# tingliu/glia

Hardware: AMD Instinct MI355X
Metric: region_merges_per_sec (higher is better)
Workload: dtype u32 labels / f32 image / f64 statistics and features

## Files before the change

glia_amd/csrc/api.cpp:

```cpp
#include <algorithm>
#include <atomic>
#include <chrono>
#include <cmath>
#include <cstdio>
#include <cstdlib>
#include <cstring>
#include <limits>
#include <mutex>
#include <unordered_map>

#include "bc_features.hpp"
#include "forest.hpp"
#include "rmap_order.hpp"
#include "hmt_internal.hpp"

namespace glia {

static thread_local std::string g_err;
void set_error(const std::string& msg) { g_err = msg; }

static const char* const kOptionKeys[] = {"GLIA_HMT_PB_WINDOW", "GLIA_HMT_PB_BATCH", "GLIA_HMT_WINCAP", "GLIA_HMT_REBASE", "GLIA_HMT_HORIZON",
                                          "GLIA_HMT_FORCE_TREE", "GLIA_HMT_HELPERS", "GLIA_HMT_TRACE", "GLIA_HMT_LIBM", "GLIA_HMT_BC_NOCOMMON",
                                          "GLIA_HMT_BC_GENERIC", "GLIA_HMT_DEBUG", "GLIA_HMT_MAXITERS", "GLIA_HMT_MINCAP"};
static std::mutex g_opt_mu;
static std::unordered_map<std::string, std::string> g_opt;
static bool g_opt_init = false;
static void opt_init_locked() {
  if (g_opt_init) return;
  for (const char* k : kOptionKeys) if (const char* e = getenv(k)) g_opt[k] = e;
  g_opt_init = true;
}
static bool opt_known(const char* key) { for (const char* k : kOptionKeys) if (!strcmp(k, key)) return true; return false; }
bool option(const char* key, std::string* value) {
  std::lock_guard<std::mutex> lock(g_opt_mu);
  opt_init_locked();
  auto it = g_opt.find(key);
  if (it == g_opt.end()) return false;
  if (value) *value = it->second;
  return true;
}
int set_option(const char* key, const char* value) {
  if (!key || !opt_known(key)) { set_error(std::string("set_option: unknown option ") + (key ? key : "(null)")); return GLIA_HMT_ERR_ARG; }
  std::lock_guard<std::mutex> lock(g_opt_mu);
  opt_init_locked();
  if (value) g_opt[key] = value; else g_opt.erase(key);
  return GLIA_HMT_OK;
}

static float ceil_f32(double d) {
  if (std::isinf(d) || std::isnan(d)) return (float)d;
  float f = (float)d;
  if ((double)f < d) f = std::nextafterf(f, std::numeric_limits<float>::infinity());
  return f;
}
static float floor_f32(double d) {
  if (std::isinf(d) || std::isnan(d)) return (float)d;
  float f = (float)d;
  if ((double)f > d) f = std::nextafterf(f, -std::numeric_limits<float>::infinity());
  return f;
}
static uint32_t next_pow2(uint64_t v) {
  uint64_t p = 1;
  while (p < v) p <<= 1;
  return (uint32_t)std::min<uint64_t>(p, 1ull << 31);
}

HistSpec make_hist_spec(int bins, double lo, double hi) {
  HistSpec h;
  h.bins = bins;
  double interval = (hi - lo) / bins;
  double b = 0.0;
  for (int i = 0; i < GLIA_HMT_MAX_BINS; ++i) {
    if (i < bins) { b = (i == 0) ? interval : b + interval; h.fb[i] = ceil_f32(b); }
    else h.fb[i] = std::numeric_limits<float>::infinity();
  }
  h.lo_f = floor_f32(lo);
  h.hi_f = ceil_f32(hi);
  return h;
}


static LibmSel probe_host_libm() {
  std::vector<double> xs;
  uint64_t s = 0x9E3779B97F4A7C15ull;
  auto next = [&]() { s ^= s << 13; s ^= s >> 7; s ^= s << 17; return s; };
  for (int i = 0; i < 6000; ++i) { const uint64_t n = 1 + next() % 100000, c = 1 + next() % n; xs.push_back((double)c / (double)n); }
  for (int i = 0; i < 3000; ++i) xs.push_back(1.0 + ((double)(int64_t)(next() % 2000001) - 1000000.0) * 1e-7);
  for (int i = 0; i < 3000; ++i) xs.push_back(std::ldexp(1.0 + (double)(next() >> 12) * 0x1p-52, (int)(next() % 120) - 60));
  for (int e = -1074; e < 1024; e += 37) xs.push_back(std::ldexp(1.0, e));
  LibmSel sel = {kLibmDevice, kLibmDevice, kLibmDevice};
  bool l2 = true, ls = true, lf = true, ps = true, pf = true;
  for (double x : xs) {
    volatile double vx = x;
    const double h2 = std::log2(vx), h1 = std::log(vx);
    l2 = l2 && glibc::as_u64(h2) == glibc::as_u64(glibc::log2_sse2(x));
    ls = ls && glibc::as_u64(h1) == glibc::as_u64(glibc::log_sse2(x));
    lf = lf && glibc::as_u64(h1) == glibc::as_u64(glibc::log_fma(x));
  }
  for (int i = 0; i < 12000; ++i) {
    const double x = i < 4000 ? (double)(i + 1) : (double)(1 + next() % (i < 8000 ? (1ull << 24) : (1ull << 40)));
    volatile double vx = x, vy = 1.5;
    const uint64_t h = glibc::as_u64(std::pow(vx, vy));
    ps = ps && h == glibc::as_u64(glibc::pow_sse2(x, 1.5));
    pf = pf && h == glibc::as_u64(glibc::pow_fma(x, 1.5));
  }
  if (l2) sel.log2_variant = kLibmSse2;
  if (lf) sel.log_variant = kLibmFma; else if (ls) sel.log_variant = kLibmSse2;
  if (pf) sel.pow_variant = kLibmFma; else if (ps) sel.pow_variant = kLibmSse2;
  std::string ov;
  if (option("GLIA_HMT_LIBM", &ov)) {
    const char* e = ov.c_str();
    const int v = !strcmp(e, "sse2") ? kLibmSse2 : !strcmp(e, "fma") ? kLibmFma : kLibmDevice;
    sel.log_variant = v; sel.log2_variant = v == kLibmFma ? kLibmSse2 : v; sel.pow_variant = v;
  }
  return sel;
}

}

namespace glia {
GLIA_DECLARE_GREEDY_BC(greedy_bc) {
  auto* fn = &greedy_bc_generic;
  const bool common = cfg.K == 1 && cfg.n_region == 1 && cfg.n_rlabel == 0 && cfg.n_boundary == 1 && !cfg.use_hist && !cfg.use_log &&
                      !cfg.use_simple && !option("GLIA_HMT_BC_NOCOMMON");
  if (cfg.libm_log2 == kLibmSse2 && cfg.libm_log == kLibmFma && cfg.libm_pow == kLibmFma) fn = common ? &greedy_bc_fma_common : &greedy_bc_fma;
  else if (cfg.libm_log2 == kLibmSse2 && cfg.libm_log == kLibmSse2 && cfg.libm_pow == kLibmSse2) fn = common ? &greedy_bc_sse2_common : &greedy_bc_sse2;
  if (option("GLIA_HMT_BC_GENERIC")) fn = &greedy_bc_generic;
  const int rc = fn(rag, cfg, clf, stream, req, out);
  return req.init_only ? rc : finish_merge_order(rc, out->order.data(), out->n, (uint32_t)rag.R, stream);
}
}

using namespace glia;

#include "api_types.hpp"

static std::atomic<int> g_live_contexts{0};

static int free_tables(glia_hmt_ctx* c) {
  if (c->rkeys) GLIA_HIP_TRY(hipFree(c->rkeys));
  if (c->rrec) GLIA_HIP_TRY(hipFree(c->rrec));
  if (c->pkeys) GLIA_HIP_TRY(hipFree(c->pkeys));
  if (c->prec) GLIA_HIP_TRY(hipFree(c->prec));
  c->rkeys = nullptr; c->rrec = nullptr; c->pkeys = nullptr; c->prec = nullptr;
  c->rcap = c->pcap = 0;
  return GLIA_HMT_OK;
}

static int ensure_tables(glia_hmt_ctx* c, uint32_t rcap, uint32_t pcap) {
  if (rcap <= c->rcap && pcap <= c->pcap) return GLIA_HMT_OK;
  rcap = std::max(rcap, c->rcap);
  pcap = std::max(pcap, c->pcap);
  int rc = free_tables(c);
  if (rc) return rc;
  GLIA_HIP_TRY(hipMalloc(&c->rkeys, sizeof(uint32_t) * (size_t)rcap));
  GLIA_HIP_TRY(hipMalloc(&c->rrec, sizeof(uint32_t) * kRegionWords * (size_t)rcap));
  GLIA_HIP_TRY(hipMalloc(&c->pkeys, sizeof(unsigned long long) * (size_t)pcap));
  GLIA_HIP_TRY(hipMalloc(&c->prec, sizeof(uint32_t) * kPairWords * (size_t)pcap));
  GLIA_HIP_TRY(hipMemsetAsync(c->rkeys, 0, sizeof(uint32_t) * (size_t)rcap, c->stream));
  GLIA_HIP_TRY(hipMemsetAsync(c->rrec, 0, sizeof(uint32_t) * kRegionWords * (size_t)rcap, c->stream));
  GLIA_HIP_TRY(hipMemsetAsync(c->pkeys, 0, sizeof(unsigned long long) * (size_t)pcap, c->stream));
  GLIA_HIP_TRY(hipMemsetAsync(c->prec, 0, sizeof(uint32_t) * kPairWords * (size_t)pcap, c->stream));
  c->rcap = rcap;
  c->pcap = pcap;
  return GLIA_HMT_OK;
}

static int clear_tables(glia_hmt_ctx* c) {
  GLIA_HIP_TRY(hipMemsetAsync(c->rkeys, 0, sizeof(uint32_t) * (size_t)c->rcap, c->stream));
  GLIA_HIP_TRY(hipMemsetAsync(c->rrec, 0, sizeof(uint32_t) * kRegionWords * (size_t)c->rcap, c->stream));
  GLIA_HIP_TRY(hipMemsetAsync(c->pkeys, 0, sizeof(unsigned long long) * (size_t)c->pcap, c->stream));
  GLIA_HIP_TRY(hipMemsetAsync(c->prec, 0, sizeof(uint32_t) * kPairWords * (size_t)c->pcap, c->stream));
  return GLIA_HMT_OK;
}

extern "C" {
// ... 427 lines not shown
int glia_hmt_rag_from_arrays(glia_hmt_ctx* c, const glia_hmt_rag* like, int64_t n_regions, const uint32_t* d_region_label,
                             const uint32_t* d_region_rec, int64_t n_pairs, const uint32_t* d_pair_a, const uint32_t* d_pair_b,
                             const uint32_t* d_pair_rec, glia_hmt_rag** out) {
  if (!c || !like || !out || n_regions < 0 || n_pairs < 0) { set_error("rag_from_arrays: invalid argument"); return GLIA_HMT_ERR_ARG; }
  GLIA_HIP_TRY(hipSetDevice(c->device));
  glia_hmt_rag* rag = new glia_hmt_rag(*like);
  rag->ctx = c;
  rag->d_folded = nullptr; rag->vol = VolumeRef();
  rag->arr = RagArrays();
  rag->arr.R = n_regions; rag->arr.P = n_pairs;
  auto dup = [&](uint32_t** dst, const uint32_t* src, size_t n) -> int {
    GLIA_HIP_TRY(hipMalloc(dst, sizeof(uint32_t) * (n ? n : 1)));
    if (n) GLIA_HIP_TRY(hipMemcpyAsync(*dst, src, sizeof(uint32_t) * n, hipMemcpyDeviceToDevice, c->stream));
    return GLIA_HMT_OK;
  };
  int rc;
  if ((rc = dup(&rag->arr.d_rlabel, d_region_label, (size_t)n_regions)) || (rc = dup(&rag->arr.d_rrec, d_region_rec, (size_t)n_regions * kRegionWords)) ||
      (rc = dup(&rag->arr.d_pa, d_pair_a, (size_t)n_pairs)) || (rc = dup(&rag->arr.d_pb, d_pair_b, (size_t)n_pairs)) ||
      (rc = dup(&rag->arr.d_prec, d_pair_rec, (size_t)n_pairs * kPairWords))) { glia_hmt_rag_free(rag); return rc; }
  rag->arr.K = 1; rag->arr.c_rrec[0] = rag->arr.d_rrec; rag->arr.c_prec[0] = rag->arr.d_prec;
  for (int k = 0; k < kMaxChannels; ++k) rag->arr.c_bins[k] = like->arr.c_bins[k];
  rag->arr.c_bins[0] = rag->bins;
  GLIA_HIP_TRY(hipStreamSynchronize(c->stream));
  *out = rag;
  return GLIA_HMT_OK;
}

void glia_hmt_rag_free(glia_hmt_rag* r) {
  if (!r) return;
  (void)hipSetDevice(r->ctx->device);
  (void)hipFree(r->arr.d_rlabel); (void)hipFree(r->arr.d_rrec);
  (void)hipFree(r->arr.d_pa); (void)hipFree(r->arr.d_pb); (void)hipFree(r->arr.d_prec);
  for (int k = 1; k < r->arr.K; ++k) { (void)hipFree(r->arr.c_rrec[k]); (void)hipFree(r->arr.c_prec[k]); }
  if (r->arr.d_pv_off) (void)hipFree(r->arr.d_pv_off);
  if (r->arr.d_pv) (void)hipFree(r->arr.d_pv);
  if (r->d_folded) (void)hipFree(r->d_folded);
  delete r;
}

int64_t glia_hmt_rag_num_regions(const glia_hmt_rag* r) { return r ? r->arr.R : -1; }
int64_t glia_hmt_rag_num_pairs(const glia_hmt_rag* r) { return r ? r->arr.P : -1; }

int glia_hmt_rag_last_pass(const glia_hmt_rag* r, double* ms, double* bytes) {
  if (!r) return GLIA_HMT_ERR_ARG;
  if (ms) *ms = r->pass_ms;
  if (bytes) *bytes = r->alg_bytes;
  return GLIA_HMT_OK;
}

static double dword(const uint32_t* w) { double d; std::memcpy(&d, w, 8); return d; }

int glia_hmt_rag_export_regions(const glia_hmt_rag* r, uint32_t* h_label, int64_t* h_count, int64_t* h_border,
                                int64_t* h_lo, int64_t* h_hi, double* h_sum, double* h_sumsq, double* h_min,
                                double* h_max, int64_t* h_hist, int64_t* h_first) {
  if (!r) return GLIA_HMT_ERR_ARG;
  GLIA_HIP_TRY(hipSetDevice(r->ctx->device));
  const int64_t R = r->arr.R;
  std::vector<uint32_t> lab(R), rec((size_t)R * kRegionWords);
  if (R) {
    GLIA_HIP_TRY(hipMemcpy(lab.data(), r->arr.d_rlabel, sizeof(uint32_t) * R, hipMemcpyDeviceToHost));
    GLIA_HIP_TRY(hipMemcpy(rec.data(), r->arr.d_rrec, sizeof(uint32_t) * kRegionWords * R, hipMemcpyDeviceToHost));
  }
  for (int64_t i = 0; i < R; ++i) {
    const uint32_t* w = &rec[(size_t)i * kRegionWords];
    if (h_label) h_label[i] = lab[i];
    if (h_count) h_count[i] = w[R_CNT];
    if (h_border) h_border[i] = w[R_BORDER];
    for (int d = 0; d < 3; ++d) {
      if (h_lo) h_lo[3 * i + d] = (int64_t)(0x7fffffffu - w[R_LO + d]);
      if (h_hi) h_hi[3 * i + d] = (int64_t)w[R_HI + d] - 1;
    }
    if (h_sum) h_sum[i] = dword(&w[R_SUM]);
    if (h_sumsq) h_sumsq[i] = dword(&w[R_SQ]);
    if (h_min) h_min[i] = (double)ord_float(~w[R_MIN]);
    if (h_max) h_max[i] = (double)ord_float(w[R_MAX]);
    if (h_hist) for (int b = 0; b < r->bins; ++b) h_hist[i * r->bins + b] = w[R_HIST + b];
    if (h_first) { unsigned long long f; std::memcpy(&f, &w[R_FIRST], 8); h_first[i] = (int64_t)~f; }
  }
  return GLIA_HMT_OK;
}

int glia_hmt_rag_export_pairs(const glia_hmt_rag* r, uint32_t* h_a, uint32_t* h_b, int64_t* h_count, double* h_sum,
                              double* h_sumsq, double* h_min, double* h_max, int64_t* h_hist, int64_t* h_thr) {
  if (!r) return GLIA_HMT_ERR_ARG;
  GLIA_HIP_TRY(hipSetDevice(r->ctx->device));
  const int64_t P = r->arr.P;
  std::vector<uint32_t> a(P), b(P), rec((size_t)P * kPairWords);
  if (P) {
    GLIA_HIP_TRY(hipMemcpy(a.data(), r->arr.d_pa, sizeof(uint32_t) * P, hipMemcpyDeviceToHost));
    GLIA_HIP_TRY(hipMemcpy(b.data(), r->arr.d_pb, sizeof(uint32_t) * P, hipMemcpyDeviceToHost));
    GLIA_HIP_TRY(hipMemcpy(rec.data(), r->arr.d_prec, sizeof(uint32_t) * kPairWords * P, hipMemcpyDeviceToHost));
  }
  for (int64_t i = 0; i < P; ++i) {
    const uint32_t* w = &rec[(size_t)i * kPairWords];
    if (h_a) h_a[i] = a[i];
    if (h_b) h_b[i] = b[i];
    if (h_count) h_count[i] = w[P_CNT];
    if (h_sum) h_sum[i] = dword(&w[P_SUM]);
    if (h_sumsq) h_sumsq[i] = dword(&w[P_SQ]);
    if (h_min) h_min[i] = (double)ord_float(~w[P_MIN]);
    if (h_max) h_max[i] = (double)ord_float(w[P_MAX]);
    if (h_hist) for (int k = 0; k < r->bins; ++k) h_hist[i * r->bins + k] = w[P_HIST + k];
    if (h_thr) for (int k = 0; k < r->nthr; ++k) h_thr[i * r->nthr + k] = w[P_THR + k];
  }
  return GLIA_HMT_OK;
}

static int order_to_keys(const glia_hmt_rag* rag, const MergeResult& res, const char* who, bool contour_keys, int64_t capacity,
                         uint32_t* h_order, double* h_sal, int64_t* n_merges) {
  const int64_t R = rag->arr.R, n = res.n;
  if (n > capacity) { set_error(std::string(who) + ": output capacity too small"); return GLIA_HMT_ERR_CAPACITY; }
  std::vector<uint32_t> lab((size_t)R);
  GLIA_HIP_TRY(hipMemcpy(lab.data(), rag->arr.d_rlabel, sizeof(uint32_t) * R, hipMemcpyDeviceToHost));
  uint32_t maxKey = lab[R - 1];
  if (contour_keys) GLIA_HIP_TRY(hipMemcpy(&maxKey, rag->arr.d_pa + (rag->arr.P - 1), sizeof(uint32_t), hipMemcpyDeviceToHost));
  for (int64_t i = 0; i < 3 * n; ++i) {
    const uint32_t id = res.order[i];
    h_order[i] = id < (uint32_t)R ? lab[id] : maxKey + 1u + (id - (uint32_t)R);
  }
  std::copy(res.sal.begin(), res.sal.begin() + n, h_sal);
  *n_merges = n;
  return GLIA_HMT_OK;
}

int glia_hmt_merge_order_pb(glia_hmt_ctx* c, glia_hmt_rag* rag, int type, uint32_t* h_order, double* h_sal,
                            int64_t capacity, int64_t* n_merges) {
  if (!c || !rag || !h_order || !h_sal || !n_merges || rag->ctx != c) {
    set_error("merge_order_pb: invalid argument");
    return GLIA_HMT_ERR_ARG;
  }
  if (type == 3 && rag->only_contour) {
    set_error("merge_order_pb: the median x min-size linkage needs region sizes (only_contour = 0)");
    return GLIA_HMT_ERR_ARG;
  }
  if ((type == 1 || type == 3) && !rag->vol.lab && !rag->arr.d_pv_off) {
    set_error("merge_order_pb: median linkage needs the volumes the RAG was built from (whole-volume build) or a map that carries its "
              "boundary values (glia_hmt_rag_build_distributed with with_values)");
    return GLIA_HMT_ERR_UNSUPPORTED;
  }
  if (type != 1 && type != 2 && type != 3) {
    set_error("Error: unsupported boundary stats type...");
    return GLIA_HMT_ERR_ARG;
  }
  GLIA_HIP_TRY(hipSetDevice(c->device));
  *n_merges = 0;
  if (rag->arr.R == 0 || rag->arr.P == 0) return GLIA_HMT_OK;
  PbRequest req;
  if (type == 1 || type == 3) req.median_of = &rag->vol;
  req.size_weight = type == 3;
  MergeResult res;
  const int rc = greedy_mean(rag->arr, c->stream, req, &res);
  if (rc) return rc;
  rag->ms_table = res.ms_table; rag->ms_loop = res.ms_loop; rag->n_scored = res.n_scored;
  return order_to_keys(rag, res, "merge_order_pb", rag->only_contour, capacity, h_order, h_sal, n_merges);
}

static int upload_forest(const HostForest& hf, glia_hmt_forest* f, int slot, hipStream_t stream) {
  std::vector<PackedNode> nodes;
  std::vector<int> roots;
  int rc = pack_forest(hf, &nodes, &roots);
  if (rc) return rc;
  PackedNode* d_nodes = nullptr;
  int* d_roots = nullptr;
  GLIA_HIP_TRY(hipMalloc(&d_nodes, sizeof(PackedNode) * nodes.size()));
  f->allocs.push_back(d_nodes);
  GLIA_HIP_TRY(hipMalloc(&d_roots, sizeof(int) * roots.size()));
  f->allocs.push_back(d_roots);
  GLIA_HIP_TRY(hipMemcpyAsync(d_nodes, nodes.data(), sizeof(PackedNode) * nodes.size(), hipMemcpyHostToDevice, stream));
  GLIA_HIP_TRY(hipMemcpyAsync(d_roots, roots.data(), sizeof(int) * roots.size(), hipMemcpyHostToDevice, stream));
  std::vector<PackedTriple> lines;
  std::vector<int> proots;
  rc = pack_forest_triples(hf, &lines, &proots);
  if (rc) return rc;
  PackedTriple* d_lines = nullptr;
  int* d_proots = nullptr;
  GLIA_HIP_TRY(hipMalloc(&d_lines, sizeof(PackedTriple) * lines.size()));
  f->allocs.push_back(d_lines);
  GLIA_HIP_TRY(hipMalloc(&d_proots, sizeof(int) * proots.size()));
  f->allocs.push_back(d_proots);
  GLIA_HIP_TRY(hipMemcpyAsync(d_lines, lines.data(), sizeof(PackedTriple) * lines.size(), hipMemcpyHostToDevice, stream));
  GLIA_HIP_TRY(hipMemcpyAsync(d_proots, proots.data(), sizeof(int) * proots.size(), hipMemcpyHostToDevice, stream));
  GLIA_HIP_TRY(hipStreamSynchronize(stream));
  f->dc.f[slot].ntree = hf.ntree; f->dc.f[slot].nrnodes = hf.nrnodes; f->dc.f[slot].nnodes = (int)nodes.size();
  f->dc.f[slot].nodes = d_nodes; f->dc.f[slot].root = d_roots;
  f->dc.f[slot].triples = d_lines; f->dc.f[slot].troot = d_proots;
  if (hf.max_var > f->max_var) f->max_var = hf.max_var;
  return GLIA_HMT_OK;
}

int glia_hmt_forest_load(glia_hmt_ctx* c, int n_models, const char* const* paths, int predict_label,
                         const double* dist, glia_hmt_forest** out) {
  if (!c || !paths || !out || (n_models != 1 && n_models != 3)) {
    set_error("forest_load: one model, or three models with distributor arguments, expected");
    return GLIA_HMT_ERR_ARG;
  }
  if (n_models == 3 && !dist) { set_error("Error: model distributor needs 3 arguments..."); return GLIA_HMT_ERR_ARG; }
  GLIA_HIP_TRY(hipSetDevice(c->device));
  glia_hmt_forest* f = new glia_hmt_forest;
  f->device = c->device;
  memset(&f->dc, 0, sizeof(f->dc));
  f->dc.kind = 0; f->dc.n_models = n_models;
  if (dist) {
    f->dc.dim0 = (int)dist[0]; f->dc.dim1 = (int)dist[1]; f->dc.threshold = dist[2];
    if (f->dc.dim0 < 0 || f->dc.dim1 < 0) { delete f; set_error("forest_load: negative distributor dimension"); return GLIA_HMT_ERR_ARG; }
    f->max_var = std::max(f->dc.dim0, f->dc.dim1);
  }
  for (int i = 0; i < n_models; ++i) {
    HostForest hf;
    int rc = load_forest_file(paths[i], predict_label, &hf);
    if (rc == GLIA_HMT_OK) rc = upload_forest(hf, f, i, c->stream);
    if (rc) { glia_hmt_forest_free(f); return rc; }
  }
  *out = f;
  return GLIA_HMT_OK;
}

int glia_hmt_forest_file_parse(const char* path, int predict_label, int* ntree, int* nrnodes, int* nclass,
                               double* h_split, int* h_meta, int64_t capacity_nodes) {
  if (!path || !ntree || !nrnodes || !nclass) { set_error("forest_file_parse: invalid argument"); return GLIA_HMT_ERR_ARG; }
  HostForest hf;
  int rc = load_forest_file(path, predict_label, &hf);
  if (rc) return rc;
  *ntree = hf.ntree; *nrnodes = hf.nrnodes; *nclass = hf.nclass;
  const int64_t nodes = (int64_t)hf.ntree * hf.nrnodes;
  if (h_split || h_meta) {
    if (nodes > capacity_nodes) { set_error("forest_file_parse: capacity too small"); return GLIA_HMT_ERR_CAPACITY; }
    if (h_split) memcpy(h_split, hf.split.data(), sizeof(double) * nodes);
    if (h_meta) memcpy(h_meta, hf.meta.data(), sizeof(int) * 4 * nodes);
  }
  return GLIA_HMT_OK;
}

int glia_hmt_forest_stub(glia_hmt_ctx* c, int feature_index, glia_hmt_forest** out) {
  if (!c || !out || feature_index < 0) { set_error("forest_stub: invalid argument"); return GLIA_HMT_ERR_ARG; }
  glia_hmt_forest* f = new glia_hmt_forest;
  f->device = c->device;
  memset(&f->dc, 0, sizeof(f->dc));
  f->dc.kind = 1; f->dc.n_models = 1; f->dc.stub_index = feature_index; f->max_var = feature_index;
  *out = f;
  return GLIA_HMT_OK;
}

void glia_hmt_forest_free(glia_hmt_forest* f) {
  if (!f) return;
  (void)hipSetDevice(f->device);
  for (void* p : f->allocs) (void)hipFree(p);
  delete f;
}

static inline double sdivide_host(double l, double r) { return std::fabs(r) >= 2.22e-16 ? l / r : 0.0; }

static bool make_bc_cfg(const glia_hmt_rag* rag, BcCfg* c) {
  if (!rag->has_cfg) return false;
  const glia_hmt_feat_config& g = rag->cfg;
  memset(c, 0, sizeof(*c));
  c->D = rag->dim; c->T = g.n_thresholds; c->bins = rag->bins;
  c->K = rag->arr.K;
  for (int k = 0; k < kMaxChannels; ++k) c->cbins[k] = k < rag->arr.K ? rag->arr.c_bins[k] : 0;
  c->n_region = g.n_region; c->n_rlabel = g.n_rlabel; c->n_boundary = g.n_boundary;
  for (int i = 0; i < kMaxListed; ++i) { c->rc[i] = rag->map_region[i]; c->lc[i] = rag->map_rlabel[i]; c->bc[i] = rag->map_boundary[i]; }
  c->use_log = g.use_log_shape; c->use_simple = g.use_simple_features; c->use_hist = g.use_histogram_features;
  c->norm_area = g.normalizing_area; c->norm_len = g.normalizing_length;
  c->rfdim = bc_rf_dim(*c); c->bfdim = bc_bf_dim(*c); c->fdim = bc_feat_dim(*c);
  c->libm_log2 = rag->ctx->libm.log2_variant; c->libm_log = rag->ctx->libm.log_variant; c->libm_pow = rag->ctx->libm.pow_variant;
  return true;
}

static int median_extra_cols(const glia_hmt_rag* rag, const BcCfg& c) {
  if (!rag->cfg.use_median_features) return 0;
  return c.use_simple ? c.n_boundary : 4 * c.n_region + 4 * c.n_boundary;
}
static int refuse_median_in_loop(const glia_hmt_rag* rag, const char* who) {
  if (!rag->has_cfg || !rag->cfg.use_median_features) return GLIA_HMT_OK;
  set_error(std::string(who) + ": the GLIA_USE_MEDIAN_AS_FEATS layout (type/feat.hxx:677-722) is implemented for a given merge order only (glia_hmt_bc_feat): "
            "inside the greedy loop every contraction changes the value multisets of its regions and boundary sets");
  return GLIA_HMT_ERR_UNSUPPORTED;
}

int glia_hmt_feat_dim(const glia_hmt_rag* rag) {
  BcCfg c;
  if (!rag || !make_bc_cfg(rag, &c)) return -1;
  return c.fdim + median_extra_cols(rag, c);
}

static int bc_setup(glia_hmt_ctx* c, const glia_hmt_rag* rag, const glia_hmt_forest* forest, const char* who, BcCfg* cfg) {
  if (!make_bc_cfg(rag, cfg) || rag->only_contour) {
    set_error(std::string(who) + ": the region map must be built with a feature configuration and with region points");
    return GLIA_HMT_ERR_ARG;
  }
  if (forest) {
    if (int rm = refuse_median_in_loop(rag, who)) return rm;
    if (forest->max_var >= cfg->fdim) { set_error(std::string(who) + ": the classifier reads features beyond the vector"); return GLIA_HMT_ERR_ARG; }
  }
  GLIA_HIP_TRY(hipSetDevice(c->device));
  return GLIA_HMT_OK;
}
static void keep_timing(glia_hmt_rag* rag, const MergeResult& res) {
  rag->ms_table = res.ms_table; rag->ms_init = res.ms_init; rag->ms_loop = res.ms_loop; rag->n_scored = res.n_scored;
}

int glia_hmt_merge_order_bc(glia_hmt_ctx* c, glia_hmt_rag* rag, const glia_hmt_forest* forest, uint32_t* h_order,
                            double* h_sal, double* h_feats, int64_t capacity, int64_t* n_merges) {
  if (!c || !rag || !forest || !h_order || !h_sal || !n_merges || rag->ctx != c) {
    set_error("merge_order_bc: invalid argument");
    return GLIA_HMT_ERR_ARG;
  }
// ... 208 lines not shown
  }
  if (!rag->vol.lab) { set_error("boundary_confidence: needs the volumes the region map was built from (whole-volume build)"); return GLIA_HMT_ERR_UNSUPPORTED; }
  GLIA_HIP_TRY(hipSetDevice(c->device));
  const int64_t P = rag->arr.P;
  std::vector<uint32_t> pa((size_t)(P ? P : 1)), pb((size_t)(P ? P : 1));
  if (P) {
    GLIA_HIP_TRY(hipMemcpy(pa.data(), rag->arr.d_pa, sizeof(uint32_t) * P, hipMemcpyDeviceToHost));
    GLIA_HIP_TRY(hipMemcpy(pb.data(), rag->arr.d_pb, sizeof(uint32_t) * P, hipMemcpyDeviceToHost));
  }
  std::vector<float> val;
  int rc = boundary_confidence_values(n_trees, n_nodes, node_label, parent, child0, potential, pa.data(), pb.data(), P, &val);
  if (rc) return rc;
  return paint_pair_values(rag->vol, rag->arr.d_pa, rag->arr.d_pb, P, val.data(), d_out, c->stream);
}

double glia_hmt_last_transform_ms(const glia_hmt_ctx* c) { return c ? c->transform_ms : 0.0; }

int64_t glia_hmt_gen_tree(const uint32_t* h_order, int64_t n_merges, uint32_t* node_label, int32_t* parent, int32_t* child0,
                          int32_t* child1, int64_t capacity) {
  if (!h_order || !node_label || !parent || !child0 || !child1 || n_merges < 0) { set_error("gen_tree: invalid argument"); return GLIA_HMT_ERR_ARG; }
  std::unordered_map<uint32_t, int> nmap;
  int64_t ni = 0;
  auto add = [&](uint32_t label, int c0, int c1) -> int64_t {
    if (ni >= capacity) return -1;
    node_label[ni] = label; parent[ni] = -1; child0[ni] = c0; child1[ni] = c1;
    nmap.emplace(label, (int)ni);
    return ni++;
  };
  for (int64_t i = 0; i < n_merges; ++i) {
    const uint32_t x0 = h_order[3 * i], x1 = h_order[3 * i + 1], x2 = h_order[3 * i + 2];
    auto n0 = nmap.find(x0);
    int64_t i0 = n0 == nmap.end() ? add(x0, -1, -1) : n0->second;
    auto n1 = nmap.find(x1);
    int64_t i1 = n1 == nmap.end() ? add(x1, -1, -1) : n1->second;
    if (i0 < 0 || i1 < 0 || ni >= capacity) { set_error("gen_tree: output capacity too small"); return GLIA_HMT_ERR_CAPACITY; }
    parent[i0] = (int32_t)ni; parent[i1] = (int32_t)ni;
    add(x2, (int)i0, (int)i1);
  }
  return ni;
}

int glia_hmt_score_initial_edges(glia_hmt_ctx* c, glia_hmt_rag* rag, const glia_hmt_forest* forest, int64_t* n_edges,
                                 double* ms) {
  if (!c || !rag || !forest || rag->ctx != c) { set_error("score_initial_edges: invalid argument"); return GLIA_HMT_ERR_ARG; }
  BcCfg cfg;
  int rc;
  if ((rc = bc_setup(c, rag, forest, "score_initial_edges", &cfg))) return rc;
  BcRequest req;
  req.init_only = true;
  MergeResult res;
  if ((rc = greedy_bc(rag->arr, cfg, forest->dc, c->stream, req, &res))) return rc;
  keep_timing(rag, res);
  if (n_edges) *n_edges = rag->n_scored;
  if (ms) *ms = rag->ms_init;
  return GLIA_HMT_OK;
}

int glia_hmt_score_initial_edges_shard(glia_hmt_ctx* c, glia_hmt_rag* rag, const glia_hmt_forest* forest, int shard, int n_shards,
                                       double* h_scores, int64_t capacity, int64_t* n_records) {
  if (!c || !rag || !forest || rag->ctx != c || n_shards < 1 || shard < 0 || shard >= n_shards || !n_records) {
    set_error("score_initial_edges_shard: invalid argument");
    return GLIA_HMT_ERR_ARG;
  }
  BcCfg cfg;
  int rc;
  if ((rc = bc_setup(c, rag, forest, "score_initial_edges", &cfg))) return rc;
  BcRequest req;
  req.init_only = true; req.scores = h_scores != nullptr; req.shard = shard; req.n_shards = n_shards;
  MergeResult res;
  if ((rc = greedy_bc(rag->arr, cfg, forest->dc, c->stream, req, &res))) return rc;
  keep_timing(rag, res);
  *n_records = res.n;
  if (h_scores) {
    if (res.n > capacity) { set_error("score_initial_edges_shard: output capacity too small"); return GLIA_HMT_ERR_CAPACITY; }
    std::copy(res.sal.begin(), res.sal.begin() + res.n, h_scores);
  }
  return GLIA_HMT_OK;
}

int glia_hmt_bc_label(glia_hmt_ctx* c, glia_hmt_rag* rag, const uint32_t* const* d_truth, int n_truth, const uint32_t* h_order,
                      int64_t n_merges, const glia_hmt_bc_label_opts* opts, int32_t* h_labels) {
  glia_hmt_bc_label_opts o = {GLIA_HMT_BC_LABEL_F1, 0, 1.0, 0, 0};
  if (opts) o = *opts;
  if (!c || !rag || rag->ctx != c || !d_truth || n_truth < 1 || n_merges < 0 || (n_merges && (!h_order || !h_labels))) {
    set_error("bc_label: invalid argument");
    return GLIA_HMT_ERR_ARG;
  }
  for (int t = 0; t < n_truth; ++t) if (!d_truth[t]) { set_error("bc_label: null truth volume"); return GLIA_HMT_ERR_ARG; }
  if (o.metric < GLIA_HMT_BC_LABEL_F1 || o.metric > GLIA_HMT_BC_LABEL_VI) { set_error("bc_label: unknown metric"); return GLIA_HMT_ERR_ARG; }
  if (o.global_opt < 0 || o.global_opt > 2) { set_error("Error: unsupported globalOpt type..."); return GLIA_HMT_ERR_ARG; }
  if (n_truth > 1 && o.metric != GLIA_HMT_BC_LABEL_VI) { set_error("bc_label: several truth volumes need the VI metric (bc_label_vi)"); return GLIA_HMT_ERR_ARG; }
  if (o.metric == GLIA_HMT_BC_LABEL_VI && (o.tweak || o.opt_split || o.max_prec_drop < 1.0)) {
    set_error("bc_label: tweak, mpd and optSplit are options of bc_label_ri, not of bc_label_vi");
    return GLIA_HMT_ERR_ARG;
  }
  if (rag->only_contour) { set_error("bc_label: the region map must hold region points (only_contour = 0)"); return GLIA_HMT_ERR_ARG; }
  if (!rag->vol.lab) { set_error("bc_label: needs the volumes the region map was built from (whole-volume build)"); return GLIA_HMT_ERR_UNSUPPORTED; }
  const int64_t R = rag->arr.R;
  if (n_merges && n_merges >= R) { set_error("bc_label: more merges than regions"); return GLIA_HMT_ERR_ARG; }
  std::vector<uint32_t> lab((size_t)R);
  if (R) GLIA_HIP_TRY(hipMemcpy(lab.data(), rag->arr.d_rlabel, sizeof(uint32_t) * R, hipMemcpyDeviceToHost));
  std::unordered_map<uint32_t, uint32_t> id;
  id.reserve((size_t)R * 2);
  for (int64_t i = 0; i < R; ++i) id[lab[i]] = (uint32_t)i;
  std::vector<uint32_t> forced((size_t)2 * n_merges);
  std::vector<uint8_t> used((size_t)R + n_merges, 0);
  for (int64_t i = 0; i < n_merges; ++i) {
    for (int s2 = 0; s2 < 2; ++s2) {
      auto it = id.find(h_order[3 * i + s2]);
      if (it == id.end() || used[it->second]) { set_error("bc_label: merge order refers to an unknown or already merged region"); return GLIA_HMT_ERR_ARG; }
      used[it->second] = 1;
      forced[2 * i + s2] = it->second;
    }
    if (id.count(h_order[3 * i + 2])) { set_error("bc_label: merge order reuses a region key"); return GLIA_HMT_ERR_ARG; }
    id[h_order[3 * i + 2]] = (uint32_t)(R + i);
  }
  rag->bcl = glia_hmt_bc_label_timing{0, 0, 0, 0, 0, 0};
  if (n_merges == 0) return GLIA_HMT_OK;
  GLIA_HIP_TRY(hipSetDevice(c->device));
  std::vector<NodeTruthStats> st((size_t)n_truth);
  for (int t = 0; t < n_truth; ++t) {
    std::vector<TruthCount> cnt;
    float ms = 0;
    if (int rc = truth_overlap(rag->vol, rag->arr.d_rlabel, (uint32_t)R, d_truth[t], c->stream, &cnt, &ms)) return rc;
    const auto t0 = std::chrono::steady_clock::now();
    int64_t moves = 0, pairs = 0;
    node_truth_stats(cnt, (uint32_t)R, forced.data(), n_merges, &st[t], &moves, &pairs);
    rag->bcl.ms_count += ms;
    rag->bcl.ms_nodes += std::chrono::duration<double, std::milli>(std::chrono::steady_clock::now() - t0).count();
    rag->bcl.entries += (int64_t)cnt.size(); rag->bcl.moves += moves; rag->bcl.node_pairs += pairs;
  }
  const auto t1 = std::chrono::steady_clock::now();
  int rc = bc_label_rules(st, (uint32_t)R, forced.data(), n_merges, o, h_labels);
  rag->bcl.ms_rules = std::chrono::duration<double, std::milli>(std::chrono::steady_clock::now() - t1).count();
  return rc;
}

int glia_hmt_last_bc_label_timing(const glia_hmt_rag* r, glia_hmt_bc_label_timing* out) {
  if (!r || !out) return GLIA_HMT_ERR_ARG;
  *out = r->bcl;
  return GLIA_HMT_OK;
}

int glia_hmt_last_merge_timing(const glia_hmt_rag* r, double* ms_table, double* ms_init, double* ms_loop,
                               int64_t* n_scored) {
  if (!r) return GLIA_HMT_ERR_ARG;
  if (ms_table) *ms_table = r->ms_table;
  if (ms_init) *ms_init = r->ms_init;
  if (ms_loop) *ms_loop = r->ms_loop;
  if (n_scored) *n_scored = r->n_scored;
  return GLIA_HMT_OK;
}

}
```

glia_amd/csrc/api_types.hpp:

```cpp
#pragma once
#include "glibc_math.hpp"
#include "greedy_common.hpp"
#include "hmt_internal.hpp"

using namespace glia;

struct glia_hmt_ctx {
  int device = 0;
  hipStream_t stream = nullptr;
  bool own_stream = false;
  uint32_t rcap = 0, pcap = 0;
  uint32_t* rkeys = nullptr; uint32_t* rrec = nullptr;
  unsigned long long* pkeys = nullptr; uint32_t* prec = nullptr;
  uint32_t* flags = nullptr;
  hipEvent_t ev0 = nullptr, ev1 = nullptr;
  uint32_t hint_rcap = 0, hint_pcap = 0;
  double transform_ms = 0;
  int tz = kTZ;
  LibmSel libm = {kLibmDevice, kLibmDevice, kLibmDevice};
};

struct glia_hmt_rag {
  glia_hmt_ctx* ctx = nullptr;
  int dim = 3;
  int64_t dims[3] = {1, 1, 1};
  bool only_contour = false;
  int bins = 0, nthr = 0;
  RagArrays arr;
  double pass_ms = 0, alg_bytes = 0;
  double ms_table = 0, ms_init = 0, ms_loop = 0;
  glia_hmt_bc_label_timing bcl;
  int64_t n_scored = 0;
  glia_hmt_feat_config cfg;
  bool has_cfg = false;
  VolumeRef vol;
  VolumeRef slab;
  uint32_t* d_folded = nullptr;
  int map_region[GLIA_HMT_MAX_IMAGES] = {0}, map_rlabel[GLIA_HMT_MAX_IMAGES] = {0}, map_boundary[GLIA_HMT_MAX_IMAGES] = {0};
};
```

glia_amd/csrc/greedy.hip:

```cpp
#include <atomic>
#include <cstring>
#include <vector>
#include <limits>
#include <rocprim/device/device_scan.hpp>
#include <rocprim/device/device_radix_sort.hpp>
#include <rocprim/device/device_segmented_radix_sort.hpp>

#include "greedy_batch.hpp"

namespace glia {

__global__ void pq_build_level_kernel(PqTree t, int l) {
  const int lane = threadIdx.x & 63;
  uint32_t j = (blockIdx.x * blockDim.x + threadIdx.x) >> 6;
  if (j < t.lv[l].size) (void)pq_recompute_node(t, l, j, lane, true);
}

int pq_setup(DeviceBuffers& buf, PqTree& t, hipStream_t stream) {
  t.nlevels = 0;
  uint32_t n = t.nleaves;
  while (true) {
    n = (n + kFan - 1) / kFan;
    if (t.nlevels >= kMaxLevels) { set_error("greedy: edge table too large"); return GLIA_HMT_ERR_ARG; }
    PqLevel& L = t.lv[t.nlevels++];
// ... 239 lines not shown
    GLIA_HIP_TRY(hipMemcpyAsync(h_range, range, sizeof(h_range), hipMemcpyDeviceToHost, stream));
    GLIA_HIP_TRY(hipStreamSynchronize(stream));
    return GLIA_HMT_OK;
  }
  int rebaseline(WinState& ws, uint32_t n_edges, unsigned long long* ctrl, hipStream_t stream) {
    GLIA_HIP_TRY(hipMemsetAsync(counter, 0, sizeof(uint32_t), stream));
    hipLaunchKernelGGL(win_collect_kernel, dim3((n_edges + 255) / 256), dim3(256), 0, stream, ws.er, n_edges, ws.rdead, kseq, vals, counter);
    uint32_t n = 0;
    GLIA_HIP_TRY(hipMemcpyAsync(&n, counter, sizeof(uint32_t), hipMemcpyDeviceToHost, stream));
    GLIA_HIP_TRY(hipStreamSynchronize(stream));
    if (n > E0) { set_error("greedy: more live edges than initial edges (internal error)"); return GLIA_HMT_ERR_INTERNAL; }
    if (n) {
      size_t bytes = tmp_bytes;
      GLIA_HIP_TRY(rocprim::radix_sort_pairs_desc(tmp, bytes, kseq, kseq2, vals, vals2, (size_t)n, 0, 64, stream));
      hipLaunchKernelGGL(win_salkey_kernel, dim3((n + 255) / 256), dim3(256), 0, stream, ws.er, vals2, n, ksal);
      bytes = tmp_bytes;
      GLIA_HIP_TRY(rocprim::radix_sort_pairs_desc(tmp, bytes, ksal, ksal2, vals2, isort, (size_t)n, 0, 64, stream));
    }
    GLIA_HIP_TRY(hipMemsetAsync(ws.whead, 0xFF, sizeof(uint32_t) * ws.wB, stream));
    GLIA_HIP_TRY(hipMemsetAsync(ws.wcnt, 0, sizeof(uint32_t) * ws.wB, stream));
    if (n) hipLaunchKernelGGL(win_baseline_fill_kernel, dim3((n + 255) / 256), dim3(256), 0, stream, ws, n, isort, iseq);
    hipLaunchKernelGGL(win_segments_kernel, dim3((ws.wB + 1 + 255) / 256), dim3(256), 0, stream, ws, isort, n, ige);
    GLIA_HIP_TRY(hipGetLastError());
    ws.nsort = n;
    std::string renv;
    ws.rebase_after = option("GLIA_HMT_REBASE", &renv) ? strtoull(renv.c_str(), nullptr, 10) : std::max<unsigned long long>(800000ull, (unsigned long long)n / 2ull);
    ws.wch = 0;
    if (horizon_factor > 0.0 && n > 4096) {
      unsigned long long topkey = 0;
      GLIA_HIP_TRY(hipMemcpyAsync(&topkey, ksal2, sizeof(topkey), hipMemcpyDeviceToHost, stream));
      GLIA_HIP_TRY(hipStreamSynchronize(stream));
      const long long top_cell = (long long)win_cell(f64_unord(topkey), h_range[0], h_range[1], ws.wB);
      if (prev_top_cell >= 0 && n_edges > prev_ne) {
        const double d = (double)std::max<long long>(0, prev_top_cell - top_cell);
        const double delta = std::max(horizon_factor * d * (double)ws.rebase_after / (double)(n_edges - prev_ne), (double)ws.wB / 512.0);
        ws.wch = (double)top_cell > delta ? (uint32_t)((double)top_cell - delta) : 0u;
      }
      prev_top_cell = top_cell; prev_ne = n_edges;
    }
    ws.ne_base = n_edges;
    const double inf = std::numeric_limits<double>::infinity();
    ctrl[CTRL_CTHR] = (unsigned long long)(long long)(ws.wB - 1);
    memcpy(&ctrl[CTRL_TSAL], &inf, 8); ctrl[CTRL_TSEQ] = ~0ull; ctrl[CTRL_IPTR] = 0;
    return GLIA_HMT_OK;
  }
};

static int run_pb_loop(const RagArrays& rag, hipStream_t stream, const PbRequest& req, MergeResult* out) {
  const long long P = rag.P;
  const uint32_t R = (uint32_t)rag.R;
  if (R == 0 || P == 0) return GLIA_HMT_OK;
  const VolumeRef* median_of = req.median_of;
  CallEvents<3> ev;
  int rc;
  if ((rc = ev.create())) return rc;
  GLIA_HIP_TRY(hipEventRecord(ev.ev[0], stream));
  DeviceBuffers buf;
  uint32_t* flag; uint32_t* eidx; long long* partner;
  if ((rc = buf.get(&flag, P + 1, true, stream))) return rc;
  if ((rc = buf.get(&eidx, P + 1, false, stream))) return rc;
  if ((rc = buf.get(&partner, P, false, stream))) return rc;
  hipLaunchKernelGGL(edge_flags, dim3((unsigned)((P + 255) / 256)), dim3(256), 0, stream, rag.d_pa, rag.d_pb, P, flag, partner);
  if ((rc = rocprim_run(buf, stream, [&](void* t, size_t& b) {
        return rocprim::exclusive_scan(t, b, flag, eidx, 0u, (size_t)(P + 1), rocprim::plus<uint32_t>(), stream); }))) return rc;
  uint32_t E0 = 0;
  GLIA_HIP_TRY(hipMemcpyAsync(&E0, eidx + P, sizeof(uint32_t), hipMemcpyDeviceToHost, stream));
  GLIA_HIP_TRY(hipStreamSynchronize(stream));
  if (E0 == 0) return GLIA_HMT_OK;

  GreedyState st;
  memset(&st, 0, sizeof(st));
  st.R0 = R;
  const bool mincap = initial_capacities(E0, 18, 36, &st.Ecap, &st.pool_cap);
  if ((rc = buf.get(&st.adj_off, 2 * (size_t)R, true, stream))) return rc;
  if ((rc = buf.get(&st.adj_len, 2 * (size_t)R + 1, true, stream))) return rc;
  std::string o_window, o_batch, o_txt;
  const bool batch_off = option("GLIA_HMT_PB_BATCH", &o_batch) && o_batch[0] == '0';
  bool window = !median_of && !req.size_weight && !(option("GLIA_HMT_PB_WINDOW", &o_window) && o_window[0] == '0');
  WinState ws;
  memset(&ws, 0, sizeof(ws));
  GrowList edges, entries, values;
  if (window) {
    if ((rc = entries.add(buf, &ws.fpool, st.pool_cap, stream))) return rc;
    if ((rc = edges.add(buf, &ws.er, st.Ecap, stream))) return rc;
  }
  else if ((rc = entries.add(buf, &st.pool, st.pool_cap, stream))) return rc;
  if ((rc = edges.add(buf, &st.e_u, st.Ecap, stream)) || (rc = edges.add(buf, &st.e_v, st.Ecap, stream)) ||
      (rc = edges.add(buf, &st.e_posu, st.Ecap, stream)) || (rc = edges.add(buf, &st.e_posv, st.Ecap, stream)) ||
      (rc = edges.add(buf, &st.e_mean, st.Ecap, stream)) || (rc = edges.add(buf, &st.e_n, st.Ecap, stream, true)) ||
      (rc = edges.add(buf, &st.pq.leaf_sal, st.Ecap, stream)) || (rc = edges.add(buf, &st.pq.leaf_seq, st.Ecap, stream)))
    return rc;
  st.pq.nleaves = st.Ecap;
  if ((rc = buf.get(&st.rsz, 2 * (size_t)R, true, stream))) return rc;
  if ((rc = buf.get(&st.rsum, 2 * (size_t)R, true, stream))) return rc;
  st.cond_n = req.cond_n; st.cond_rpb = req.cond_rpb; st.size_weight = req.size_weight ? 1 : 0;
  st.cond_t0 = req.cond_n > 0 ? (unsigned long long)req.cond_sizes[0] : 0; st.cond_t1 = req.cond_n > 1 ? (unsigned long long)req.cond_sizes[1] : 0;
  hipLaunchKernelGGL(region_sizes, dim3((R + 255) / 256), dim3(256), 0, stream, rag.d_rrec, R, st.rsz, st.rsum);
  if ((rc = buf.get(&st.mark0, 2 * (size_t)R, true, stream))) return rc;
  if ((rc = buf.get(&st.mark1, 2 * (size_t)R, true, stream))) return rc;
  if ((rc = buf.get(&st.order, 3 * ((size_t)R + 16), false, stream))) return rc;
  if ((rc = buf.get(&st.sal_out, (size_t)R + 16, false, stream))) return rc;
  if ((rc = buf.get(&st.ctrl, 16, true, stream))) return rc;
  uint32_t* cursor;
  if ((rc = buf.get(&cursor, 2 * (size_t)R, true, stream))) return rc;

  hipLaunchKernelGGL(fill_leaves_dead, dim3((st.Ecap - E0 + 255) / 256), dim3(256), 0, stream, st.pq, E0);
  hipLaunchKernelGGL(edge_fill, dim3((unsigned)((P + 255) / 256)), dim3(256), 0, stream, rag.d_pa, rag.d_pb, rag.d_prec, P,
                     flag, eidx, partner, rag.d_rlabel, R, st, st.adj_len);
  if ((rc = rocprim_run(buf, stream, [&](void* t, size_t& b) {
        return rocprim::exclusive_scan(t, b, st.adj_len, st.adj_off, 0u, (size_t)R, rocprim::plus<uint32_t>(), stream); }))) return rc;
  if (window) hipLaunchKernelGGL(adj_fill_fat, dim3((E0 + 255) / 256), dim3(256), 0, stream, st, ws, E0, cursor);
  else hipLaunchKernelGGL(adj_fill, dim3((E0 + 255) / 256), dim3(256), 0, stream, st, E0, cursor);
  GLIA_HIP_TRY(hipGetLastError());
  unsigned long long n_values = 0;
  if (median_of) {
    if ((rc = edges.add(buf, &st.e_off, st.Ecap, stream))) return rc;
    if ((rc = buf.get(&st.rbv, 2 * (size_t)R, true, stream))) return rc;
    if ((rc = rocprim_run(buf, stream, [&](void* t, size_t& b) {
          return rocprim::exclusive_scan(t, b, st.e_n, st.e_off, 0ull, (size_t)E0 + 1, rocprim::plus<unsigned long long>(), stream); }))) return rc;
    GLIA_HIP_TRY(hipMemcpyAsync(&n_values, st.e_off + E0, sizeof(n_values), hipMemcpyDeviceToHost, stream));
    GLIA_HIP_TRY(hipStreamSynchronize(stream));
    if (n_values >= 0xFFFFFFFFull) { set_error("merge_order_pb: more than 2^32 boundary voxels (median linkage)"); return GLIA_HMT_ERR_ARG; }
    st.vals_cap = mincap ? std::max(n_values, 1ull) : n_values * 4ull + (1ull << 20);
    float* unsorted;
    if ((rc = values.add(buf, &st.vals, (size_t)st.vals_cap, stream))) return rc;
    if ((rc = buf.get(&unsorted, (size_t)n_values, false, stream))) return rc;
    uint32_t* vcursor;
    if ((rc = buf.get(&vcursor, (size_t)E0, true, stream))) return rc;
    if (median_of->lab) {
      const long long N = median_of->nx * median_of->ny * median_of->nz;
      hipLaunchKernelGGL(median_collect, dim3((unsigned)((N + 255) / 256)), dim3(256), 0, stream, *median_of, rag.d_pa, rag.d_pb, P,
                         flag, eidx, st.e_off, vcursor, unsorted);
    } else {
      if (!rag.d_pv_off) { set_error("merge_order_pb: median linkage needs the volume or the map's boundary values"); return GLIA_HMT_ERR_UNSUPPORTED; }
      if (rag.nV) hipLaunchKernelGGL(median_from_runs, dim3((unsigned)((rag.nV + 255) / 256)), dim3(256), 0, stream, rag.d_pv_off, rag.d_pv, rag.nV, rag.d_pa, rag.d_pb,
                                     (long long)P, flag, eidx, st.e_off, unsorted);
    }
    GLIA_HIP_TRY(hipGetLastError());
    if ((rc = rocprim_run(buf, stream, [&](void* t, size_t& b) {
          return rocprim::segmented_radix_sort_keys(t, b, unsorted, st.vals, (unsigned)n_values, (unsigned)E0, st.e_off, st.e_off + 1, 0, 32, stream); }))) return rc;
    hipLaunchKernelGGL(median_init, dim3((E0 + 255) / 256), dim3(256), 0, stream, st, E0);
    GLIA_HIP_TRY(hipGetLastError());
  }
  unsigned long long ctrl[CTRL_WORDS] = {};
  ctrl[CTRL_EDGES] = E0; ctrl[CTRL_ENTRIES] = 2ull * E0; ctrl[CTRL_STATUS] = ST_RUN; ctrl[CTRL_VALUES] = n_values;
  WinBaseline base;
  if (window) {
    uint32_t B = 256;
    while (B < E0 / 4 && B < (1u << 22)) B <<= 1;
    ws.wB = B; ws.R0 = R;
    ws.wcap = kWinCap; ws.wbudget = kWinBudget;
    ws.force_tree = 0;
    if (option("GLIA_HMT_FORCE_TREE", &o_txt)) ws.force_tree = strtoull(o_txt.c_str(), nullptr, 10);
    if (option("GLIA_HMT_WINCAP", &o_txt)) {
      const uint32_t c = (uint32_t)strtoul(o_txt.c_str(), nullptr, 10);
      if (c >= 16 && c <= kWinCap) { ws.wcap = c; ws.wbudget = c / 2; }
    }
    ws.order = st.order; ws.sal_out = st.sal_out; ws.ctrl = st.ctrl; ws.rsz = st.rsz; ws.rsum = st.rsum;
    ws.mark0 = st.mark0; ws.mark1 = st.mark1; ws.adj_off = st.adj_off; ws.adj_len = st.adj_len;
    ws.pool_cap = st.pool_cap; ws.Ecap = st.Ecap;
    ws.cond_n = st.cond_n; ws.cond_t0 = st.cond_t0; ws.cond_t1 = st.cond_t1; ws.cond_rpb = st.cond_rpb;
    if ((rc = base.init(buf, ws, st.pq.leaf_sal, E0, B, R, stream))) return rc;
    if (req.cond_n <= 0 && !batch_off) base.horizon_factor = option("GLIA_HMT_HORIZON", &o_txt) ? atof(o_txt.c_str()) : 0.5;
    if ((rc = base.rebaseline(ws, E0, ctrl, stream))) return rc;
  } else if ((rc = pq_setup(buf, st.pq, stream))) return rc;
  GLIA_HIP_TRY(hipMemcpyAsync(st.ctrl, ctrl, sizeof(ctrl), hipMemcpyHostToDevice, stream));
  GLIA_HIP_TRY(hipEventRecord(ev.ev[1], stream));


  st.max_iters = window ? 1ull << 22 : 1ull << 16;
  const bool trace = option("GLIA_HMT_TRACE");
  if (option("GLIA_HMT_MAXITERS", &o_txt)) st.max_iters = std::max(1ull, strtoull(o_txt.c_str(), nullptr, 10));
  const auto kernel = [&]() { return !window ? "tree" : req.cond_n > 0 ? "window" : "batch"; };
  const auto unhandled = [&]() {
    set_error(std::string("greedy: the ") + kernel() + " kernel stopped with status " + std::to_string(ctrl[CTRL_STATUS]) + ", which its driver does not handle (internal error)");
    return GLIA_HMT_ERR_INTERNAL;
  };
  while (true) {
    if (window) {
      ws.max_iters = st.max_iters;
      if (req.cond_n > 0) hipLaunchKernelGGL(greedy_window_kernel<true>, dim3(1), dim3(kGreedyThreads), 0, stream, ws);
      else if (batch_off) hipLaunchKernelGGL(greedy_window_kernel<false>, dim3(1), dim3(kGreedyThreads), 0, stream, ws);
      else hipLaunchKernelGGL(greedy_batch_kernel, dim3(1), dim3(kGreedyThreads), 0, stream, ws);
    } else if (median_of) hipLaunchKernelGGL(greedy_pb_kernel<true>, dim3(1), dim3(kGreedyThreads), 0, stream, st);
    else hipLaunchKernelGGL(greedy_pb_kernel<false>, dim3(1), dim3(kGreedyThreads), 0, stream, st);
    GLIA_HIP_TRY(hipGetLastError());
    GLIA_HIP_TRY(hipMemcpyAsync(ctrl, st.ctrl, sizeof(ctrl), hipMemcpyDeviceToHost, stream));
    GLIA_HIP_TRY(hipStreamSynchronize(stream));
    if (trace) fprintf(stderr, "[trace] merge loop launch ended: status %llu, merges %llu of %u regions, edges %llu, list entries %llu\n", ctrl[CTRL_STATUS], ctrl[CTRL_MERGES], R, ctrl[CTRL_EDGES], ctrl[CTRL_ENTRIES]);
    if (ctrl[CTRL_STATUS] == ST_DONE) break;
    switch (ctrl[CTRL_STATUS]) {
      case ST_RUN:
        if (!window) continue;
        break;
      case ST_REBASE:
        if (!window) return unhandled();
        break;
      case ST_BAD_SALIENCY: set_error("Error: invalid boundary saliency..."); return GLIA_HMT_ERR_SALIENCY;
      case ST_INTERNAL: {
        char msg[256];
        snprintf(msg, sizeof(msg), "greedy: window queue overflow or more merges than regions (internal error: merges %llu of %u regions, %llu edges of %u initial, "
                 "window %llu%s, %s kernel)", ctrl[CTRL_MERGES], R, ctrl[CTRL_EDGES], E0, ctrl[CTRL_WFILL], ctrl[CTRL_WERR] ? " overflowed" : "", kernel());
        set_error(msg);
        return GLIA_HMT_ERR_INTERNAL;
      }
      case ST_NEED_TREE:
        if (!window) return unhandled();
        entries.remove(&ws.fpool);
        edges.remove(&ws.er);
        if ((rc = entries.add(buf, &st.pool, st.pool_cap, stream))) return rc;
        hipLaunchKernelGGL(fat_to_thin, dim3((unsigned)((ctrl[CTRL_ENTRIES] + 255) / 256)), dim3(256), 0, stream, ws.fpool, st.pool, ctrl[CTRL_ENTRIES]);
        hipLaunchKernelGGL(edge_unpack, dim3((unsigned)((ctrl[CTRL_EDGES] + 255) / 256)), dim3(256), 0, stream, st, ws.er, ws.rdead, (uint32_t)ctrl[CTRL_EDGES]);
        GLIA_HIP_TRY(hipGetLastError());
        if ((rc = pq_setup(buf, st.pq, stream))) return rc;
        window = false;
        st.max_iters = 1ull << 16;
        break;
      case ST_NEED_POOL: {
        const unsigned long long ncap = st.pool_cap * 2;
        if ((rc = entries.grow(buf, (size_t)st.pool_cap, (size_t)ncap, stream))) return rc;
        st.pool_cap = ncap; ws.pool_cap = ncap;
        break;
      }
      case ST_NEED_VALUES: {
        if (!median_of) return unhandled();
        const unsigned long long ncap = st.vals_cap * 2;
        if ((rc = values.grow(buf, (size_t)ctrl[CTRL_VALUES], (size_t)ncap, stream))) return rc;
        st.vals_cap = ncap;
        break;
      }
      case ST_NEED_EDGES: {
        if (st.Ecap >= kMaxEdgeSlots) { set_error("greedy: more than 2^32 edge slots needed"); return GLIA_HMT_ERR_ARG; }
        const uint32_t ocap = st.Ecap, ncap = (uint32_t)std::min<unsigned long long>(kMaxEdgeSlots, (unsigned long long)ocap * 2ull);
        if ((rc = edges.grow(buf, ocap, ncap, stream))) return rc;
        st.Ecap = ncap; st.pq.nleaves = ncap; ws.Ecap = ncap;
        hipLaunchKernelGGL(fill_leaves_dead, dim3((ncap - ocap + 255) / 256), dim3(256), 0, stream, st.pq, ocap);
        if (!window && (rc = pq_setup(buf, st.pq, stream))) return rc;
        break;
      }
      default: return unhandled();
    }
    if (window) {
      if ((rc = base.rebaseline(ws, (uint32_t)ctrl[CTRL_EDGES], ctrl, stream))) return rc;
      GLIA_HIP_TRY(hipMemcpyAsync(st.ctrl + CTRL_CTHR, ctrl + CTRL_CTHR, 4 * sizeof(unsigned long long), hipMemcpyHostToDevice, stream));
    }
    unsigned long long zero = ST_RUN;
    GLIA_HIP_TRY(hipMemcpyAsync(st.ctrl + CTRL_STATUS, &zero, sizeof(zero), hipMemcpyHostToDevice, stream));
  }
  GLIA_HIP_TRY(hipEventRecord(ev.ev[2], stream));
  GLIA_HIP_TRY(hipEventSynchronize(ev.ev[2]));
  out->ms_table = ev.ms(0, 1); out->ms_loop = ev.ms(1, 2);
  out->n_scored = (int64_t)ctrl[CTRL_EDGES];
  return copy_merges(out, (int64_t)ctrl[CTRL_MERGES], st.order, st.sal_out);
}


static std::atomic<unsigned long long> g_internal_errors{0};
unsigned long long internal_errors() { return g_internal_errors.load(); }
void count_internal_error() { g_internal_errors.fetch_add(1); }
bool merge_order_is_consistent(const uint32_t* o, int64_t n, uint32_t R, int64_t* first_bad) {
  std::vector<uint8_t> gone(2 * (size_t)R + 1, 0);
  for (int64_t k = 0; k < n; ++k) {
    const uint32_t a = o[3 * k], b = o[3 * k + 1], c = o[3 * k + 2];
    if (k >= (int64_t)R || c != R + (uint32_t)k || a >= c || b >= c || a == b || gone[a] || gone[b]) { if (first_bad) *first_bad = k; return false; }
    gone[a] = gone[b] = 1;
  }
  return true;
}
int finish_merge_order(int rc, const uint32_t* o, int64_t n, uint32_t R, hipStream_t stream) {
  int64_t bad = -1;
  if (rc == GLIA_HMT_OK && !merge_order_is_consistent(o, n, R, &bad)) {
    set_error("greedy: merge " + std::to_string(bad) + " of " + std::to_string(n) + " joins a region that does not exist (any more) or creates the wrong one (internal error)");
    rc = GLIA_HMT_ERR_INTERNAL;
  }
  if (rc == GLIA_HMT_ERR_INTERNAL) { count_internal_error(); (void)hipStreamSynchronize(stream); }
  return rc;
}
int greedy_mean(const RagArrays& rag, hipStream_t stream, const PbRequest& req, MergeResult* out) {
  const int rc = run_pb_loop(rag, stream, req, out);
  return finish_merge_order(rc, out->order.data(), out->n, (uint32_t)rag.R, stream);
}

}
```

glia_amd/csrc/greedy_batch.hpp:

```cpp
#pragma once
#include "greedy_window.hpp"

namespace glia {
namespace {

constexpr uint32_t kBatchKill = 32;
constexpr int kMemP = 3;
constexpr uint32_t kMemMax = 192;
struct BatchShared {
  alignas(16) Key part1[kNW];
  alignas(16) Key part2[kNW];
  uint32_t nkill, kovf; alignas(16) uint32_t kill[kBatchKill];
  uint32_t byrank[kNW];
  uint32_t bitmap[kNW][64];
  uint32_t m_newcount[kNW], m_total[kNW], m_ok[kNW];
  double m_maxsal[kNW];
  uint32_t bad;
};

template <int CTRL, int ROW_MASK = 0xf>
__device__ __forceinline__ void top2_ord_step(unsigned long long& a1, unsigned long long& a2) {
  const unsigned long long b1 = dpp64<CTRL, ROW_MASK, ROW_MASK != 0xf>(a1), b2 = dpp64<CTRL, ROW_MASK, ROW_MASK != 0xf>(a2);
  const bool g = b1 > a1;
  const unsigned long long hi = g ? b1 : a1, lo = g ? a1 : b1, m2 = b2 > a2 ? b2 : a2;
  a1 = hi; a2 = lo > m2 ? lo : m2;
}
__device__ __forceinline__ void wave_top2_ord(unsigned long long& a1, unsigned long long& a2) {
  top2_ord_step<0xB1>(a1, a2);
  top2_ord_step<0x4E>(a1, a2);
  top2_ord_step<0x124>(a1, a2);
  top2_ord_step<0x128>(a1, a2);
  top2_ord_step<0x142, 0xa>(a1, a2);
  top2_ord_step<0x143, 0xc>(a1, a2);
  a1 = lane_u64(a1, 63); a2 = lane_u64(a2, 63);
}

#ifdef GLIA_HMT_PROFILE
__device__ unsigned long long g_scanprof[8];
__device__ unsigned long long g_scanfill[3][3];
#define SCAN_T(i) do { if (tid == 0) { const unsigned long long tn_ = __builtin_readcyclecounter(); g_scanprof[i] += tn_ - st_; st_ = tn_; } } while (0)
#else
#define SCAN_T(i) do {} while (0)
#endif
enum { kScanOther = 0, kScanNarrow = 1, kScanWide = 2 };
__device__ __forceinline__ void batch_scan(const WinState& st, WinShared& w, BatchShared& b, int tid, [[maybe_unused]] int from) {
#ifdef GLIA_HMT_PROFILE
  unsigned long long st_ = __builtin_readcyclecounter();
  if (tid == 0) g_scanprof[7] += 1;
#endif
  const uint32_t n = w.n < st.wcap ? w.n : st.wcap, nk = b.nkill < kBatchKill ? b.nkill : kBatchKill, kovf = b.kovf;
#ifdef GLIA_HMT_PROFILE
  if (tid == 0) g_scanfill[from][n <= 512u ? 0 : n <= 1024u ? 1 : 2] += 1;
#endif
  const uint32_t own = 64u * (uint32_t)(((tid >> 6) + (tid & 63)) & 7) + (uint32_t)(tid & 63);
  Key k1, k2;
  k1.sal = -__builtin_inf(); k1.seq = 0; k1.arg = 0; k2 = k1;
  auto pass = [&](auto nb_tag) {
    constexpr int NB = decltype(nb_tag)::value;
    unsigned long long q[NB]; uint32_t e[NB]; double sl[NB];
#pragma unroll
    for (int j = 0; j < NB; ++j) { const uint32_t i = own + (uint32_t)j * kGreedyThreads; q[j] = w.seq[i]; e[j] = w.e[i]; sl[j] = w.sal[i]; }
    const uint4 ka = *reinterpret_cast<const uint4*>(&b.kill[0]), kb = *reinterpret_cast<const uint4*>(&b.kill[4]);
    const uint32_t kl[8] = {ka.x, ka.y, ka.z, ka.w, kb.x, kb.y, kb.z, kb.w};
    SCAN_T(0);
    uint32_t deadm[NB];
#pragma unroll
    for (int j = 0; j < NB; ++j) {
      uint32_t d = 0;
#pragma unroll
      for (uint32_t t = 0; t < 8; ++t) d |= (uint32_t)(t < nk) & (uint32_t)(kl[t] == e[j]);
      deadm[j] = d;
    }
    if (nk > 8u) {
      for (uint32_t t = 8; t < nk; ++t) {
        const uint32_t kt = b.kill[t];
#pragma unroll
        for (int j = 0; j < NB; ++j) deadm[j] |= (uint32_t)(kt == e[j]);
      }
      if (kovf) {
        full_barrier();
#pragma unroll
        for (int j = 0; j < NB; ++j) {
          const uint32_t i = own + (uint32_t)j * kGreedyThreads;
          if (i < n && q[j] != 0) deadm[j] |= (uint32_t)(st.er[e[j]].seq == 0);
        }
      }
    }
#pragma unroll
    for (int j = 0; j < NB; ++j) {
      const uint32_t i = own + (uint32_t)j * kGreedyThreads;
      const bool was = (i < n) & (q[j] != 0);
      const bool live = was & (deadm[j] == 0u);
      if (was & !live) w.seq[i] = 0;
      Key c; c.sal = live ? sl[j] : -__builtin_inf(); c.seq = live ? q[j] : 0ull; c.arg = i;
      const bool b1 = better(c, k1), b2 = better(c, k2);
      k2.sal = b1 ? k1.sal : (b2 ? c.sal : k2.sal); k2.seq = b1 ? k1.seq : (b2 ? c.seq : k2.seq); k2.arg = b1 ? k1.arg : (b2 ? c.arg : k2.arg);
      k1.sal = b1 ? c.sal : k1.sal; k1.seq = b1 ? c.seq : k1.seq; k1.arg = b1 ? c.arg : k1.arg;
    }
  };
  static_assert(kWinPer == 3, "batch_scan: one pass instance per number of blocks");
  const uint32_t nu = (uint32_t)__builtin_amdgcn_readfirstlane((int)n);
  if (nu > 2u * kGreedyThreads) pass(std::integral_constant<int, 3>{});
  else if (nu > kGreedyThreads) pass(std::integral_constant<int, 2>{});
  else pass(std::integral_constant<int, 1>{});
  SCAN_T(1);
  const int lane = tid & 63;
  const unsigned long long o1 = f64_ord(k1.sal), o2 = f64_ord(k2.sal);
  unsigned long long M1 = o1, M2 = o2;
  wave_top2_ord(M1, M2);
  const unsigned long long t1 = __ballot(o1 == M1), t1l = __ballot((o1 == M1) & (k1.seq != 0ull));
  const int l1 = (int)__builtin_ctzll(t1);
  const bool win1 = lane == l1;
  Key kk; kk.sal = win1 ? k2.sal : k1.sal; kk.seq = win1 ? k2.seq : k1.seq; kk.arg = win1 ? k2.arg : k1.arg;
  const unsigned long long oc = win1 ? o2 : o1;
  const unsigned long long t2 = __ballot(oc == M2), t2l = __ballot((oc == M2) & (kk.seq != 0ull));
  Key m1, m2;
  if (__popcll(t1) == 1 || t1l == 0ull) {
    m1 = lane_key(k1, l1);
    int src = (int)__builtin_ctzll(t2);
    if (__popcll(t2) != 1 && t2l != 0ull) {
#ifdef GLIA_HMT_PROFILE
      if (tid == 0) g_scanprof[5] += 1;
#endif
      const unsigned long long ms = wave_max_u64(oc == M2 ? kk.seq : 0ull);
      src = (int)__builtin_ctzll(__ballot((oc == M2) & (kk.seq == ms)));
    }
    m2 = lane_key(kk, src);
    SCAN_T(2);
  } else {
#ifdef GLIA_HMT_PROFILE
    if (tid == 0) g_scanprof[6] += 1;
#endif
    unsigned long long S1 = o1 == M1 ? k1.seq : 0ull, S2 = o2 == M1 ? k2.seq : 0ull;
    wave_top2_ord(S1, S2);
    const int w1 = (int)__builtin_ctzll(__ballot((o1 == M1) & (k1.seq == S1)));
    const bool winr = lane == w1;
    Key kc; kc.sal = winr ? k2.sal : k1.sal; kc.seq = winr ? k2.seq : k1.seq; kc.arg = winr ? k2.arg : k1.arg;
    const unsigned long long occ = winr ? o2 : o1;
    m1 = lane_key(k1, w1);
    m2 = lane_key(kc, (int)__builtin_ctzll(__ballot((occ == M1) & (kc.seq == S2))));
    SCAN_T(3);
  }
  if ((tid & 63) == 0) { b.part1[tid >> 6] = m1; b.part2[tid >> 6] = m2; }
  full_barrier();
  SCAN_T(4);
  if (tid == 0) { b.nkill = 0; b.kovf = 0; }
}

#ifdef GLIA_HMT_PROFILE
__device__ unsigned long long g_wideprof[8];
#define WIDE_T(i) do { if (tid == 0) { const unsigned long long tn_ = __builtin_readcyclecounter(); g_wideprof[i] += tn_ - wt_; wt_ = tn_; } } while (0)
#else
#define WIDE_T(i) do {} while (0)
#endif
__device__ __forceinline__ uint32_t batch_contract_wide(const WinState& st, WinShared& w, WinWork& s, BatchShared& b, int tid, uint32_t slot, double rootsal,
                                                      unsigned long long k, unsigned long long ne, unsigned long long pool_used, double smin, double scale, uint32_t* newcount_out) {
  const uint32_t e = w.e[slot], r0 = w.u[slot], r1 = w.v[slot];
  const uint2 h0r = w.hu[slot], h1r = w.hv[slot];
  const uint32_t wn_now = w.n;
  const uint32_t off0 = h0r.x, len0 = h0r.y, off1 = h1r.x, len1 = h1r.y;
  const uint32_t total = len0 + len1;
  const uint32_t r2 = st.R0 + (uint32_t)k;
  const uint32_t r2off = (uint32_t)pool_used;
#ifdef GLIA_HMT_PROFILE
  unsigned long long wt_ = __builtin_readcyclecounter();
#endif
  lds_barrier();
  WIDE_T(0);
  if (tid == 0) {
    w.seq[slot] = 0;
    st.order[3 * k + 0] = r0; st.order[3 * k + 1] = r1; st.order[3 * k + 2] = r2;
    st.sal_out[k] = rootsal;
    st.er[e].seq = 0;
    st.rdead[r0] = 1; st.rdead[r1] = 1;
  }
  const bool small = total <= kMarkMax;
  win_stage_lists(st, s, tid, e, off0, len0, off1, len1, small);
  if (small) lds_barrier(); else full_barrier();
  WIDE_T(1);
  if (wn_now + total > st.wcap && wn_now > st.wcap / 2u) win_compact(w, tid, st.wcap);
  WIDE_T(2);
  const WinTau tau = {w.cthr, w.tsal, w.tseq, smin, scale};
  const uint32_t nwork = small ? s.nitems : total;
  const uint32_t lenR2 = small ? nwork : 0u;
  bool bad = false;
  uint32_t pend_e = kNone, pend_old = kNone;
  auto rounds = [&](auto small_tag) {
    constexpr bool SMALL = decltype(small_tag)::value;
    for (uint32_t base = 0; base < nwork; base += kGreedyThreads) {
      const uint32_t i = base + tid;
      if (i >= nwork) break;
      FatEntry f0, f1;
      bool h0, h1;
      uint32_t rs;
      if (!win_match<SMALL>(st, s, i, e, off0, len0, off1, &rs, &h0, &h1, &f0, &f1)) continue;
      const uint32_t idx = atomicAdd(&s.newcount, 1u);
      const uint32_t newE = (uint32_t)ne + idx;
      double first;
      int second;
      if (mean_link(h0, f0.mean, (int)f0.n, h1, f1.mean, (int)f1.n, &first, &second)) bad = true;
      const uint32_t offRs = f0.off, posRs = f0.pos, lenRs = f0.len;
      if (h0 && h1) st.fpool[offRs + f1.pos].eid = kNone;
      const unsigned long long seq = update_seq(k, rs, r0, h0);
      const double sal = -first;
      store_new_edge(st, newE, rs, r2, posRs, idx, first, second, sal, seq, offRs, lenRs, r2off, lenR2);
      win_queue_edge<true>(st, w, tau, newE, sal, seq, rs, r2, make_uint2(offRs, lenRs), make_uint2(r2off, lenR2), pend_e, pend_old);
      if (h0) win_retire_edge<true, false, kBatchKill>(st, tau, f0.eid, -f0.mean, &b.nkill, b.kill, &b.kovf);
      if (h1) win_retire_edge<true, false, kBatchKill>(st, tau, f1.eid, -f1.mean, &b.nkill, b.kill, &b.kovf);
    }
  };
  if (small) rounds(std::true_type{}); else rounds(std::false_type{});
  if (bad) b.bad = 1;
  WIDE_T(3);
  if (small) lds_barrier(); else full_barrier();
  WIDE_T(4);
  const uint32_t newcount = s.newcount;
  if (!small) win_complete_r2(st, tid, (uint32_t)ne, r2off, newcount);
  if (!small) for (uint32_t i = tid; i < (w.n < st.wcap ? w.n : st.wcap); i += kGreedyThreads) if (w.v[i] == r2) w.hv[i].y = newcount;
  if (pend_e != kNone) st.er[pend_e].next = pend_old;
  if (tid == 0) { st.adj_off[r2] = r2off; st.adj_len[r2] = newcount; }
  lds_barrier();
  WIDE_T(5);
  if (tid == 0) { s.nitems = 0; s.newcount = 0; }
  *newcount_out = newcount;
  return total;
}

__global__ __launch_bounds__(kGreedyThreads) void greedy_batch_kernel(WinState st) {
  __shared__ WinShared w;
  __shared__ WinWork s;
  __shared__ BatchShared b;
  const int tid = threadIdx.x, lane = tid & 63, wave = tid >> 6;
  unsigned long long k = st.ctrl[CTRL_MERGES], ne = st.ctrl[CTRL_EDGES], pool_used = st.ctrl[CTRL_ENTRIES];
  uint32_t status = ST_RUN;
  win_enter(st, w, s, tid);
  if (tid == 0) { b.nkill = 0; b.kovf = 0; b.bad = 0; }
  b.bitmap[wave][lane] = 0;
  if (tid < kNW) { Key z; z.sal = -__builtin_inf(); z.seq = 0; z.arg = 0; b.part1[tid] = z; b.part2[tid] = z; }
  full_barrier();
  const double smin = st.wrange[0], scale = st.wrange[1];
  uint32_t pend_e = kNone, pend_old = kNone;
  constexpr uint32_t kTab = kMarkSlots / kNW;
  uint32_t* const tk = &s.mk[wave * kTab]; uint32_t* const t0 = &s.mv0[wave * kTab]; uint32_t* const t1 = &s.mv1[wave * kTab];
  static_assert(sizeof(s.stage) >= (size_t)kNW * kTab * 20, "per-wave staging");
  uint32_t* const sg_eid = reinterpret_cast<uint32_t*>(&s.stage[0]) + wave * kTab;
  uint32_t* const sg_n = reinterpret_cast<uint32_t*>(&s.stage[0]) + (kNW + wave) * kTab;
  uint32_t* const sg_pos = reinterpret_cast<uint32_t*>(&s.stage[0]) + (2 * kNW + wave) * kTab;
  double* const sg_mean = reinterpret_cast<double*>(reinterpret_cast<uint32_t*>(&s.stage[0]) + 3 * kNW * kTab) + wave * kTab;
#ifdef GLIA_HMT_PROFILE
  unsigned long long bph[8] = {0, 0, 0, 0, 0, 0, 0, 0}, blast = __builtin_readcyclecounter(), brounds = 0, bmembers = 0, bvalid = 0, bwide = 0, bcut_sal = 0, bcut_dep = 0;
  unsigned long long bw_n[4] = {0, 0, 0, 0}, bw_cyc[4] = {0, 0, 0, 0}, bw_ent[4] = {0, 0, 0, 0}, bw_new[4] = {0, 0, 0, 0};
  unsigned long long bsel[2] = {0, 0}, bsel_n[2] = {0, 0};
#define BPH0(wide) do { if (tid == 0) { unsigned long long tn = __builtin_readcyclecounter(); bph[0] += tn - blast; bsel[wide] += tn - blast; bsel_n[wide] += 1; blast = tn; } } while (0)
#define BPH(i) do { if (tid == 0) { unsigned long long tn = __builtin_readcyclecounter(); bph[i] += tn - blast; blast = tn; } } while (0)
#else
#define BPH(i) do {} while (0)
#define BPH0(wide) do {} while (0)
#endif

  for (unsigned long long it = 0; it < st.max_iters; ++it) {
    if (ne - st.ne_base > st.rebase_after) { status = ST_REBASE; break; }
    const int gi = lane >> 3, gj = lane & 7;
    const Key A = b.part1[gi], B = b.part1[gj], C = b.part2[gi];
    const unsigned long long beats = __ballot(better(A, B)), under = __ballot(better(C, B));
    const unsigned long long col = 0x0101010101010101ull << gj;
    const uint32_t rank = (uint32_t)__popcll(beats & col);
    const bool cand_ok = B.seq != 0 && (under & col) == 0;
    if (gi == 0 && cand_ok) b.byrank[rank] = (uint32_t)gj;
    const unsigned long long okmask = __ballot(gi == 0 && cand_ok);
    const uint32_t M = (uint32_t)__popcll(okmask);
    if (M == 0) {
      BPH(5);
      if (pend_e != kNone) { st.er[pend_e].next = pend_old; pend_e = kNone; }
      if (st.force_tree && k >= st.force_tree) { status = ST_NEED_TREE; break; }
      const int r = win_reload(st, w, tid, reinterpret_cast<double*>(&s.stage[0]), reinterpret_cast<unsigned long long*>(&s.stage[0]) + kSelMax);
      BPH(6);
      if (r == 1) { status = ST_DONE; break; }
      if (r == 2) { status = ST_NEED_TREE; break; }
      if (r == 3) { status = ST_REBASE; break; }
      batch_scan(st, w, b, tid, kScanOther);
      continue;
    }
    const unsigned long long minemask = __ballot(gi == 0 && cand_ok && rank == (uint32_t)wave);
    const bool member = minemask != 0;
    const int cj = member ? (int)__builtin_ctzll(minemask) : 0;
    const Key me = b.part1[cj];
    const uint32_t slot = me.arg;
    const uint32_t e = w.e[slot], r0 = w.u[slot], r1 = w.v[slot];
    const uint2 h0r = w.hu[slot], h1r = w.hv[slot];
    const uint32_t off0 = h0r.x, len0 = h0r.y, off1 = h1r.x, len1 = h1r.y;
    const uint32_t total = len0 + len1;
    if (k >= (unsigned long long)st.R0) { status = ST_INTERNAL; break; }
    const unsigned long long firstmask = __ballot(gi == 0 && cand_ok && rank == 0u);
    const Key top = b.part1[__builtin_ctzll(firstmask)];
    const uint2 th0 = w.hu[top.arg], th1 = w.hv[top.arg];
    const uint32_t top_total = th0.y + th1.y;
    BPH0(top_total > kMemMax ? 1 : 0);
    if (top_total > kMemMax) {
      if (ne + top_total > st.Ecap) { status = ST_NEED_EDGES; break; }
      if (pool_used + top_total > st.pool_cap) { status = ST_NEED_POOL; break; }
      uint32_t newcount = 0;
#ifdef GLIA_HMT_PROFILE
      const unsigned long long tw0 = __builtin_readcyclecounter();
#endif
      const uint32_t tt = batch_contract_wide(st, w, s, b, tid, top.arg, top.sal, k, ne, pool_used, smin, scale, &newcount);
      if (b.bad) { status = ST_BAD_SALIENCY; break; }
      k += 1; ne += newcount; pool_used += tt;
#ifdef GLIA_HMT_PROFILE
      bwide += 1;
      { const int cls = tt <= 512u ? 0 : tt <= kMarkMax ? 1 : tt <= 8192u ? 2 : 3; bw_n[cls] += 1; bw_cyc[cls] += __builtin_readcyclecounter() - tw0; bw_ent[cls] += tt; bw_new[cls] += newcount; }
#endif
      batch_scan(st, w, b, tid, kScanWide);
      if (w.spill_ord) { if (pend_e != kNone) { st.er[pend_e].next = pend_old; pend_e = kNone; } win_evict(st, w, tid); batch_scan(st, w, b, tid, kScanOther); }
      BPH(4);
      continue;
    }
    const bool narrow = member && total <= kMemMax;
    b.bitmap[wave][lane] = 0;
    FatEntry fe[kMemP];
    bool act[kMemP], side1[kMemP];
    uint32_t h[kMemP];
#pragma unroll
    for (int p = 0; p < kMemP; ++p) {
      const uint32_t i = (uint32_t)lane + 64u * (uint32_t)p;
      const bool inlist = narrow && i < total;
      side1[p] = i >= len0;
      fe[p].eid = kNone; fe[p].rs = 0; fe[p].n = 0; fe[p].pos = 0; fe[p].off = 0; fe[p].len = 0; fe[p].mean = 0.0;
      if (inlist) fe[p] = st.fpool[side1[p] ? off1 + (i - len0) : off0 + i];
      act[p] = inlist;
    }
    if (pend_e != kNone) { st.er[pend_e].next = pend_old; pend_e = kNone; }
#pragma unroll
    for (int p = 0; p < kMemP; ++p) {
      act[p] = act[p] && fe[p].eid != e && fe[p].eid != kNone;
      h[p] = (fe[p].rs * 2654435761u) >> 24;
      if (act[p]) {
        while (true) {
          const uint32_t old = atomicCAS(&tk[h[p]], 0u, fe[p].rs + 1u);
          if (old == 0u || old == fe[p].rs + 1u) break;
          h[p] = (h[p] + 1u) & (kTab - 1u);
        }
        if (side1[p]) {
          t1[h[p]] = 1u;
          sg_eid[h[p]] = fe[p].eid; sg_n[h[p]] = fe[p].n; sg_pos[h[p]] = fe[p].pos; sg_mean[h[p]] = fe[p].mean;
        } else t0[h[p]] = 1u;
        atomicOr(&b.bitmap[wave][(fe[p].rs >> 5) & 63u], 1u << (fe[p].rs & 31u));
      }
    }
    if (narrow && lane == 0) { atomicOr(&b.bitmap[wave][(r0 >> 5) & 63u], 1u << (r0 & 31u)); atomicOr(&b.bitmap[wave][(r1 >> 5) & 63u], 1u << (r1 & 31u)); }
    asm volatile("s_waitcnt lgkmcnt(0)" ::: "memory");
    bool owner[kMemP], both[kMemP];
    uint32_t p_eid[kMemP], p_n[kMemP], p_pos[kMemP];
    double p_mean[kMemP];
#pragma unroll
    for (int p = 0; p < kMemP; ++p) {
      const uint32_t m0 = act[p] ? t0[h[p]] : 0u, m1 = act[p] ? t1[h[p]] : 0u;
      owner[p] = act[p] && (!side1[p] || m0 == 0u);
      both[p] = owner[p] && !side1[p] && m1 != 0u;
      p_eid[p] = sg_eid[h[p]]; p_n[p] = sg_n[h[p]]; p_pos[p] = sg_pos[h[p]]; p_mean[p] = sg_mean[h[p]];
    }
#pragma unroll
    for (int p = 0; p < kMemP; ++p) if (act[p]) { tk[h[p]] = 0u; t0[h[p]] = 0u; t1[h[p]] = 0u; }
    double first[kMemP]; int second[kMemP]; uint32_t idx[kMemP];
    bool bad = false;
    uint32_t newcount = 0;
    double mx = -__builtin_inf();
#pragma unroll
    for (int p = 0; p < kMemP; ++p) {
      const bool h0 = owner[p] && !side1[p], h1 = owner[p] && (side1[p] || both[p]);
      bad = mean_link(h0, fe[p].mean, (int)fe[p].n, h1, both[p] ? p_mean[p] : fe[p].mean, both[p] ? (int)p_n[p] : (int)fe[p].n, &first[p], &second[p]) || bad;
      const double f = first[p];
      const unsigned long long ownmask = __ballot(owner[p]);
      idx[p] = newcount + (uint32_t)__popcll(ownmask & ((1ull << lane) - 1ull));
      newcount += (uint32_t)__popcll(ownmask);
      mx = (owner[p] && -f > mx) ? -f : mx;
    }
#pragma unroll
    for (int d = 32; d >= 1; d >>= 1) { const double o = __shfl_xor(mx, d); mx = o > mx ? o : mx; }
    if (lane == 0) { b.m_newcount[wave] = narrow ? newcount : 0u; b.m_total[wave] = narrow ? total : 0xFFFFFFFFu; b.m_maxsal[wave] = mx; }
    if (bad) b.bad = 1;
    const uint32_t wn_round = w.n;
    lds_barrier();
    BPH(1);
    if (b.bad) { status = ST_BAD_SALIENCY; break; }
    uint32_t V, ne_off, pool_off, my_ne, my_pool;
    {
      const uint32_t j = (uint32_t)lane & 7u;
      const Key kj = b.part1[b.byrank[j]];
      const uint32_t u = w.u[kj.arg], v = w.v[kj.arg];
      const uint32_t tj = b.m_total[j], nj = b.m_newcount[j];
      double pm = -__builtin_inf();
      uint32_t hit = 0, pre_n = 0, pre_t = 0;
#pragma unroll
      for (uint32_t i = 0; i < (uint32_t)kNW; ++i) {
        const double ms = b.m_maxsal[i];
        const uint32_t bu = b.bitmap[i][(u >> 5) & 63u], bv = b.bitmap[i][(v >> 5) & 63u];
        const uint32_t ti = b.m_total[i], ni = b.m_newcount[i];
        if (i < j) { pm = ms > pm ? ms : pm; hit |= ((bu >> (u & 31u)) | (bv >> (v & 31u))) & 1u; pre_n += ni; pre_t += ti; }
      }
      const bool okj = j < M && tj != 0xFFFFFFFFu && (j == 0u || (kj.sal > pm && hit == 0u));
      const uint32_t okbits = (uint32_t)(__ballot(lane < kNW && okj) & 0xFFull);
      V = (uint32_t)__builtin_ctz(~okbits);
#ifdef GLIA_HMT_PROFILE
      if (V < M) { const uint32_t cutsal = (uint32_t)(__ballot(lane < kNW && j == V && !(kj.sal > pm)) & 0xFFull); if (cutsal) bcut_sal += 1; else bcut_dep += 1; }
#endif
      my_ne = (uint32_t)__builtin_amdgcn_readlane((int)pre_n, wave); my_pool = (uint32_t)__builtin_amdgcn_readlane((int)pre_t, wave);
      const uint32_t last = V - 1u;
      ne_off = (uint32_t)__shfl((int)(pre_n + nj), (int)last); pool_off = (uint32_t)__shfl((int)(pre_t + tj), (int)last);
    }
    const uint32_t sum_tot = pool_off;
    if (ne + sum_tot > st.Ecap) { status = ST_NEED_EDGES; break; }
    if (pool_used + sum_tot > st.pool_cap) { status = ST_NEED_POOL; break; }
    bool popped = false;
    if (wn_round + ne_off > st.wcap && wn_round > st.wcap / 2u) {
      if ((uint32_t)wave < V && lane == 0) w.seq[slot] = 0;
      popped = true;
      lds_barrier();
      win_compact(w, tid, st.wcap);
    }
    const WinTau tau = {w.cthr, w.tsal, w.tseq, smin, scale};
    BPH(2);
    if ((uint32_t)wave < V) {
      const unsigned long long kk = k + (unsigned long long)wave;
      const uint32_t r2 = st.R0 + (uint32_t)kk;
      const uint32_t r2off = (uint32_t)pool_used + my_pool;
      if (lane == 0) {
        if (!popped) w.seq[slot] = 0;
        st.order[3 * kk + 0] = r0; st.order[3 * kk + 1] = r1; st.order[3 * kk + 2] = r2;
        st.sal_out[kk] = me.sal;
        st.er[e].seq = 0;
        st.rdead[r0] = 1; st.rdead[r1] = 1;
        st.adj_off[r2] = r2off; st.adj_len[r2] = newcount;
      }
#pragma unroll
      for (int p = 0; p < kMemP; ++p) {
        if (!owner[p]) continue;
        const bool h0 = !side1[p];
        const uint32_t rs = fe[p].rs;
        const uint32_t newE = (uint32_t)ne + my_ne + idx[p];
        const uint32_t offRs = fe[p].off, posRs = fe[p].pos, lenRs = fe[p].len;
        if (both[p]) st.fpool[offRs + p_pos[p]].eid = kNone;
        const unsigned long long seq = update_seq(kk, rs, r0, h0);
        const double sal = -first[p];
        store_new_edge(st, newE, rs, r2, posRs, idx[p], first[p], second[p], sal, seq, offRs, lenRs, r2off, newcount);
        win_queue_edge<true>(st, w, tau, newE, sal, seq, rs, r2, make_uint2(offRs, lenRs), make_uint2(r2off, newcount), pend_e, pend_old);
        win_retire_edge<true, false, kBatchKill>(st, tau, fe[p].eid, -fe[p].mean, &b.nkill, b.kill, &b.kovf);
        if (both[p]) win_retire_edge<true, false, kBatchKill>(st, tau, p_eid[p], -p_mean[p], &b.nkill, b.kill, &b.kovf);
      }
    }
    lds_barrier();
    BPH(3);
#ifdef GLIA_HMT_PROFILE
    brounds += 1; bmembers += M; bvalid += V;
#endif
    k += V; ne += ne_off; pool_used += pool_off;
    batch_scan(st, w, b, tid, kScanNarrow);
    if (w.spill_ord) { if (pend_e != kNone) { st.er[pend_e].next = pend_old; pend_e = kNone; } win_evict(st, w, tid); batch_scan(st, w, b, tid, kScanOther); }
    BPH(4);
  }
#ifdef GLIA_HMT_PROFILE
  if (tid == 0) printf("[batch profile] merges %llu: select %llu  compute %llu  validate %llu  commit %llu  scan %llu  loop-top %llu  reload %llu (cycles); rounds %llu candidates %llu committed %llu (cut by saliency %llu, by adjacency %llu) wide %llu\n",
                       k, bph[0], bph[1], bph[2], bph[3], bph[4], bph[5], bph[6], brounds, bmembers, bvalid, bcut_sal, bcut_dep, bwide);
  if (tid == 0) printf("[batch profile] scan phases (cumulative cycles, wave 0): loads %llu  compare %llu  top2 %llu  top2 with a tied best %llu  barrier %llu  calls %llu  tied second %llu  tied best %llu\n",
                       g_scanprof[0], g_scanprof[1], g_scanprof[2], g_scanprof[3], g_scanprof[4], g_scanprof[7], g_scanprof[5], g_scanprof[6]);
  if (tid == 0) printf("[batch profile] scan fill (cumulative; n <= 512, <= 1024, more): after reload/evict %llu %llu %llu  after narrow round %llu %llu %llu  after wide %llu %llu %llu\n",
                       g_scanfill[0][0], g_scanfill[0][1], g_scanfill[0][2], g_scanfill[1][0], g_scanfill[1][1], g_scanfill[1][2], g_scanfill[2][0], g_scanfill[2][1], g_scanfill[2][2]);
  if (tid == 0) printf("[batch profile] loop top (this launch): narrow rounds %llu cycles %llu  wide pops %llu cycles %llu\n", bsel_n[0], bsel[0], bsel_n[1], bsel[1]);
  if (tid == 0) printf("[batch profile] wide phases (cumulative cycles): entry-barrier %llu  lists+table %llu  compact %llu  main loop (wave 0) %llu  loop barrier %llu  tail %llu\n",
                       g_wideprof[0], g_wideprof[1], g_wideprof[2], g_wideprof[3], g_wideprof[4], g_wideprof[5]);
  if (tid == 0) printf("[batch profile] wide by entries (<=512, <=1408, <=8192, more): n %llu %llu %llu %llu  cycles %llu %llu %llu %llu  entries %llu %llu %llu %llu  new edges %llu %llu %llu %llu\n",
                       bw_n[0], bw_n[1], bw_n[2], bw_n[3], bw_cyc[0], bw_cyc[1], bw_cyc[2], bw_cyc[3], bw_ent[0], bw_ent[1], bw_ent[2], bw_ent[3], bw_new[0], bw_new[1], bw_new[2], bw_new[3]);
#endif
  if (pend_e != kNone) st.er[pend_e].next = pend_old;
  full_barrier();
  win_leave(st, w, tid, k, ne, pool_used, status);
}

}
}
```

glia_amd/csrc/greedy_tree.hpp:

```cpp
#pragma once
#include "greedy_common.hpp"

namespace glia {

struct GreedyState {
  uint32_t R0;
  uint32_t* adj_off;
  uint32_t* adj_len;
  uint2* pool;
  unsigned long long pool_cap;
  uint32_t Ecap;
  uint32_t *e_u, *e_v, *e_posu, *e_posv;
  double* e_mean;
  int* e_n;
  float* vals;
  unsigned long long vals_cap;
  unsigned long long* e_off;
  unsigned long long* rbv;
  int size_weight;
  PqTree pq;
  int cond_n; unsigned long long cond_t0, cond_t1; double cond_rpb;
  unsigned long long* rsz;
  double* rsum;
  uint32_t *mark0, *mark1;
  uint32_t* order;
  double* sal_out;
  unsigned long long* ctrl;
  unsigned long long max_iters;
};
enum { CTRL_MERGES = 0, CTRL_EDGES = 1, CTRL_ENTRIES = 2,
       CTRL_STATUS = 3, CTRL_VALUES = 4,
       CTRL_CTHR = 5, CTRL_TSAL = 6, CTRL_TSEQ = 7, CTRL_IPTR = 8,
       CTRL_WERR = 9, CTRL_WFILL = 10, CTRL_WORDS = 11 };

namespace {

__device__ __forceinline__ bool mean_link(bool h0, double m0, int n0, bool h1, double m1, int n1, double* first, int* second) {
  double f = 0.0;
  int sc = 0;
  if (h0) { f += m0 * n0; sc += n0; }
  if (h1) { f += m1 * n1; sc += n1; }
  f = sdivide(f, (double)sc, 0.0);
  *first = f; *second = sc;
  return f == -1.0;
}
__device__ __forceinline__ unsigned long long update_seq(unsigned long long k, uint32_t rs, uint32_t r0, bool h0) {
  const uint32_t cat = rs < r0 ? 0u : (h0 ? 1u : 2u);
  return ((k + 1ull) << 32) | ((unsigned long long)cat << 30) | rs;
}

constexpr uint32_t kMarkSlots = 2048;
constexpr uint32_t kMarkMax = 1408;
struct Shared {
  uint32_t r0, r1, e, stop, len0, len1, off0, off1, newcount, reject;
  PqWork pq;
  uint32_t mk[kMarkSlots], mv0[kMarkSlots], mv1[kMarkSlots];
  uint32_t items[kMarkMax], nitems;
};
constexpr uint32_t kMergeTile = 1024;
struct MedianJobs {
  uint32_t n;
  uint32_t newE[kGreedyThreads], e0[kGreedyThreads], e1[kGreedyThreads];
  unsigned long long off[kGreedyThreads + 1];
  uint32_t toff[kGreedyThreads + 1];
  uint32_t tjob[kGreedyThreads], ta0[kGreedyThreads], ta1[kGreedyThreads];
  uint32_t na[kGreedyThreads], nb[kGreedyThreads];
  unsigned long long oa[kGreedyThreads], ob[kGreedyThreads];
  float med[kGreedyThreads];
  float buf[kGreedyThreads / 64][2 * kMergeTile + 64];
};
struct NoJobs {
  uint32_t n, newE[1], e0[1], e1[1], toff[2], tjob[1], ta0[1], ta1[1], na[1], nb[1];
  unsigned long long off[2], oa[1], ob[1];
  float med[1];
  float buf[kGreedyThreads / 64][2];
};

__device__ __forceinline__ uint32_t run_rank(const float* a, uint32_t n, float v, bool strict) {
  uint32_t lo = 0, hi = n;
  while (lo < hi) {
    const uint32_t mid = (lo + hi) >> 1;
    const float x = a[mid];
    if (strict ? (x < v) : (x <= v)) lo = mid + 1; else hi = mid;
  }
  return lo;
}

__device__ __forceinline__ uint32_t merge_split(const float* A, uint32_t na, const float* B, uint32_t nb, uint32_t d) {
  uint32_t lo = d > nb ? d - nb : 0u, hi = d < na ? d : na;
  while (lo < hi) {
    const uint32_t mid = (lo + hi) >> 1;
    if (A[mid] <= B[d - 1u - mid]) lo = mid + 1; else hi = mid;
  }
  return lo;
}
__device__ __forceinline__ void wave_lds_sync() {
  __builtin_amdgcn_fence(__ATOMIC_RELEASE, "wavefront");
  __builtin_amdgcn_wave_barrier();
  __builtin_amdgcn_fence(__ATOMIC_ACQUIRE, "wavefront");
}

template <bool MEDIAN>
__global__ __launch_bounds__(kGreedyThreads) void greedy_pb_kernel(GreedyState st) {
  __shared__ Shared s;
  __shared__ typename std::conditional<MEDIAN, MedianJobs, NoJobs>::type jobs;
  const int tid = threadIdx.x;
  unsigned long long k = st.ctrl[CTRL_MERGES], ne = st.ctrl[CTRL_EDGES], pool_used = st.ctrl[CTRL_ENTRIES], vals_used = st.ctrl[CTRL_VALUES];
  uint32_t status = ST_RUN;
  if (tid == 0) { s.pq.wln[0] = s.pq.wln[1] = 0; s.pq.ovf = 0; s.pq.spill = 0; s.nitems = 0; }
  for (int i = tid; i < kSetSlots; i += blockDim.x) { s.pq.set[0][i] = 0; s.pq.set[1][i] = 0; }
  for (uint32_t i = tid; i < kMarkSlots; i += blockDim.x) { s.mk[i] = 0; s.mv0[i] = 0; s.mv1[i] = 0; }
  const PqTree& pq = st.pq;
  constexpr uint32_t kTopLds = MEDIAN ? 1u : kTopMax;
  __shared__ Key s_topk[kTopLds];
  Key* topk = (!MEDIAN && pq.nlevels >= 2 && pq.lv[pq.nlevels - 1].size <= kTopLds) ? s_topk : nullptr;
  if (topk) pq_top_load<kGreedyThreads>(pq, topk, tid);
  full_barrier();
  pq_top<kGreedyThreads>(pq, s.pq, tid, topk);

#ifdef GLIA_HMT_PROFILE
  unsigned long long tph[6] = {0, 0, 0, 0, 0, 0}, tlast = __builtin_readcyclecounter();
  unsigned long long tb[4] = {0, 0, 0, 0}, nb[4] = {0, 0, 0, 0}, db[4] = {0, 0, 0, 0}, titer = tlast;
#define PH(i) do { if (tid == 0) { unsigned long long tn = __builtin_readcyclecounter(); tph[i] += tn - tlast; tlast = tn; } } while (0)
#else
#define PH(i) do {} while (0)
#endif
  for (unsigned long long it = 0; it < st.max_iters; ++it) {
    PH(5);
    if (tid == 0) {
      const Key root = pq_root<kGreedyThreads>(s.pq);
      s.stop = ST_RUN;
      s.newcount = 0;
      s.reject = 0;
      if (root.seq == 0) s.stop = ST_DONE;
      else {
        uint32_t e = root.arg;
        s.e = e; s.r0 = st.e_u[e]; s.r1 = st.e_v[e];
        if (st.cond_n > 0) {
          unsigned long long sz0 = st.rsz[s.r0], sz1 = st.rsz[s.r1];
          double su0 = st.rsum[s.r0], su1 = st.rsum[s.r1];
          if (sz0 > sz1) { unsigned long long t = sz0; sz0 = sz1; sz1 = t; double d = su0; su0 = su1; su1 = d; }
          bool ok = sz0 < st.cond_t0;
          if (!ok && st.cond_n > 1) {
            if (sz0 < st.cond_t1 && sdivide(su0, (double)sz0, 0.0) > st.cond_rpb) ok = true;
            if (!ok && sz1 < st.cond_t1 && sdivide(su1, (double)sz1, 0.0) > st.cond_rpb) ok = true;
          }
          if (!ok) { s.reject = 1; pq.leaf_seq[e] = 0; pq_touch(pq, s.pq, 0, 0, e);  }
        }
        const uint32_t len0 = st.adj_len[s.r0], len1 = st.adj_len[s.r1], off0 = st.adj_off[s.r0], off1 = st.adj_off[s.r1];
        const unsigned long long z0 = st.rsz[s.r0], z1 = st.rsz[s.r1];
        const double w0 = st.rsum[s.r0], w1 = st.rsum[s.r1];
        const unsigned long long b0 = MEDIAN ? st.rbv[s.r0] : 0ull, b1 = MEDIAN ? st.rbv[s.r1] : 0ull;
        const int en = MEDIAN ? st.e_n[e] : 0;
        s.len0 = len0; s.len1 = len1; s.off0 = off0; s.off1 = off1;
        unsigned long long tot = (unsigned long long)len0 + len1;
        if (s.reject) {}
        else if (ne + tot > st.Ecap) s.stop = ST_NEED_EDGES;
        else if (pool_used + tot > st.pool_cap) s.stop = ST_NEED_POOL;
        else if (MEDIAN && vals_used + b0 + b1 > st.vals_cap) s.stop = ST_NEED_VALUES;
        else {
          if (MEDIAN) st.rbv[st.R0 + (uint32_t)k] = b0 + b1 - 2ull * (unsigned long long)en;
          st.order[3 * k + 0] = s.r0; st.order[3 * k + 1] = s.r1; st.order[3 * k + 2] = st.R0 + (uint32_t)k;
          st.sal_out[k] = root.sal;
          st.rsz[st.R0 + (uint32_t)k] = z0 + z1;
          st.rsum[st.R0 + (uint32_t)k] = w0 + w1;
        }
      }
    }
    full_barrier();
    PH(0);
    if (s.stop != ST_RUN) { status = s.stop; break; }
    if (s.reject) { pq_propagate<kGreedyThreads>(pq, s.pq, tid, topk); continue; }
    const uint32_t r0 = s.r0, e = s.e, len0 = s.len0, len1 = s.len1, off0 = s.off0, off1 = s.off1;
    const uint32_t r2 = st.R0 + (uint32_t)k;
    const uint32_t total = len0 + len1;
    const uint32_t r2off = (uint32_t)pool_used;
    const bool small = total <= kMarkMax;

    for (uint32_t i = tid; i < total; i += kGreedyThreads) {
      const bool side1 = i >= len0;
      const uint2 pe = st.pool[side1 ? off1 + (i - len0) : off0 + i];
      const uint32_t eid = pe.x, rs = pe.y;
      if (eid == e || eid == kNone) continue;
      if (small) {
        uint32_t h = (rs * 2654435761u) >> 21;
        while (true) {
// ... 220 lines not shown
```

glia_amd/csrc/greedy_window.hpp:

```cpp
#pragma once
#include "greedy_tree.hpp"

namespace glia {

struct __attribute__((aligned(16))) FatEntry {
  uint32_t eid;
  uint32_t rs;
  uint32_t n;
  uint32_t pos;
  uint32_t off;
  uint32_t len;
  double mean;
};

namespace {

struct __attribute__((aligned(16))) EdgeRec {
  uint32_t u, v, posu, posv;
  double mean; int n; uint32_t next;
  uint2 hu, hv;
  double sal; unsigned long long seq;
};
static_assert(sizeof(EdgeRec) == 64, "EdgeRec layout");
struct WinState {
  EdgeRec* er; FatEntry* fpool;
  uint32_t* whead;
  uint32_t* wcnt;
  const uint32_t* isort; const unsigned long long* isort_seq;
  const uint32_t* ige;
  const double* wrange;
  uint32_t* order; double* sal_out; unsigned long long* ctrl;
  unsigned long long* rsz; double* rsum; uint32_t *mark0, *mark1, *adj_off, *adj_len;
  unsigned long long pool_cap, max_iters, cond_t0, cond_t1;
  double cond_rpb;
  uint32_t R0, Ecap, wB, nsort;
  unsigned long long ne_base, rebase_after;
  uint32_t wcap, wbudget;
  int cond_n;
  uint32_t wch;
  uint8_t* rdead;
  unsigned long long force_tree;
};
constexpr uint32_t kWinCap = 1536;
constexpr uint32_t kWinBudget = 768;
constexpr uint32_t kWinMinLoad = 192;
constexpr uint32_t kWinMinPartial = 96;
constexpr uint32_t kKillMax = 8;
constexpr int kNW = kGreedyThreads / 64;
constexpr int kWinPer = (int)(kWinCap / kGreedyThreads);
static_assert(kWinPer * kGreedyThreads == (int)kWinCap, "window capacity");
struct WinShared {
  double sal[kWinCap];
  unsigned long long seq[kWinCap];
  uint32_t e[kWinCap], u[kWinCap], v[kWinCap];
  uint2 hu[kWinCap], hv[kWinCap];
  int cthr; uint32_t iptr;
  double tsal; unsigned long long tseq;
  alignas(16) uint32_t n;
  uint32_t nk, kovf, pad0;
  alignas(16) uint32_t kill[kKillMax];
  alignas(16) Key part[kNW];
  uint32_t touched[2][64];
  uint32_t wsum[kNW];
  uint32_t bcast, maxcell, err, need_tree;
  double psal; unsigned long long pseq;
  unsigned long long spill_ord;
};
struct WinWork {
  uint32_t mk[kMarkSlots], mv0[kMarkSlots], mv1[kMarkSlots];
  uint32_t items[kMarkMax], newidx[kMarkMax], nitems, newcount, bad;
  FatEntry stage[kMarkMax];
};

__host__ __device__ __forceinline__ uint32_t win_cell(double sal, double smin, double scale, uint32_t B) {
  double t = (sal - smin) * scale;
  t = t > 0.0 ? t : 0.0;
  return t >= (double)(B - 1u) ? B - 1u : (uint32_t)t;
}
__device__ __forceinline__ bool win_above(int cthr, double tsal, unsigned long long tseq, int cell, double sal, unsigned long long seq) {
  return cell > cthr || (cell == cthr && (sal > tsal || (sal == tsal && seq > tseq)));
}

__device__ __forceinline__ uint32_t block_scan_incl(uint32_t v, uint32_t* wsum, int tid, uint32_t* total) {
  const int lane = tid & 63, wave = tid >> 6;
  uint32_t x = v;
#pragma unroll
  for (int d = 1; d < 64; d <<= 1) { const uint32_t y = (uint32_t)__shfl_up((int)x, d); if (lane >= d) x += y; }
  full_barrier();
  if (lane == 63) wsum[wave] = x;
  full_barrier();
  uint32_t base = 0, tot = 0;
#pragma unroll
  for (int i = 0; i < kNW; ++i) { const uint32_t s = wsum[i]; if (i < wave) base += s; tot += s; }
  *total = tot;
  return base + x;
}

__device__ __forceinline__ void win_put(WinShared& w, uint32_t slot, double sal, unsigned long long seq, uint32_t e, uint32_t u, uint32_t v, uint2 hu, uint2 hv) {
  w.sal[slot] = sal; w.seq[slot] = seq; w.e[slot] = e; w.u[slot] = u; w.v[slot] = v; w.hu[slot] = hu; w.hv[slot] = hv;
}
__device__ __forceinline__ void win_take(const WinState& st, WinShared& w, uint32_t e, const EdgeRec& r) {
  if (r.seq != 0) {
    const uint32_t slot = atomicAdd(&w.n, 1u);
    if (slot < st.wcap) win_put(w, slot, r.sal, r.seq, e, r.u, r.v, r.hu, r.hv); else w.err = 1;
  }
}

__device__ __forceinline__ void win_scan(const WinState& st, WinShared& w, int tid, uint32_t r2, uint32_t r2len) {
  const uint4 hd = *reinterpret_cast<const uint4*>(&w.n);
  const uint4 k0 = *reinterpret_cast<const uint4*>(&w.kill[0]), k1 = *reinterpret_cast<const uint4*>(&w.kill[4]);
  unsigned long long q[kWinPer]; uint32_t e[kWinPer], v[kWinPer]; double sl[kWinPer];
#pragma unroll
  for (int j = 0; j < kWinPer; ++j) { const uint32_t i = (uint32_t)tid + (uint32_t)j * kGreedyThreads; q[j] = w.seq[i]; e[j] = w.e[i]; v[j] = w.v[i]; sl[j] = w.sal[i]; }
  const uint32_t n = hd.x, nk = hd.y < kKillMax ? hd.y : kKillMax;
  const uint32_t kl[kKillMax] = {k0.x, k0.y, k0.z, k0.w, k1.x, k1.y, k1.z, k1.w};
  Key k;
  k.sal = -__builtin_inf(); k.seq = 0; k.arg = 0;
#pragma unroll
  for (int j = 0; j < kWinPer; ++j) {
    const uint32_t i = (uint32_t)tid + (uint32_t)j * kGreedyThreads;
    bool live = i < n && q[j] != 0;
    bool dead = false;
    if (nk) {
#pragma unroll
      for (uint32_t t = 0; t < kKillMax; ++t) dead = dead || (t < nk && kl[t] == e[j]);
    }
    if (live && hd.z) dead = dead || st.er[e[j]].seq == 0;
    if (live && dead) { w.seq[i] = 0; live = false; }
    if (live && v[j] == r2) w.hv[i].y = r2len;
    Key c; c.sal = live ? sl[j] : -__builtin_inf(); c.seq = live ? q[j] : 0ull; c.arg = i;
    if (better(c, k)) k = c;
  }
  k = wave_max(k);
  if ((tid & 63) == 0) w.part[tid >> 6] = k;
  lds_barrier();
  if (tid == 0) { w.nk = 0; w.kovf = 0; }
}
__device__ __forceinline__ Key win_root(const WinShared& w, int lane) {
  static_assert(kNW == 8, "win_root");
  Key k = w.part[lane & (kNW - 1)];
  key_max_step<0xB1>(k); key_max_step<0x4E>(k);
  const Key a = lane_key(k, 0), b = lane_key(k, 4);
  return better(b, a) ? b : a;
}

__device__ __forceinline__ uint32_t win_compact(WinShared& w, int tid, uint32_t cap = kWinCap) {
  double sal[kWinPer]; unsigned long long seq[kWinPer]; uint32_t e[kWinPer], u[kWinPer], v[kWinPer]; uint2 hu[kWinPer], hv[kWinPer];
  uint32_t live = 0;
  const uint32_t n = w.n < cap ? w.n : cap;
#pragma unroll
  for (int j = 0; j < kWinPer; ++j) {
    const uint32_t i = (uint32_t)tid * kWinPer + j;
    seq[j] = i < n ? w.seq[i] : 0ull;
    sal[j] = w.sal[i]; e[j] = w.e[i]; u[j] = w.u[i]; v[j] = w.v[i]; hu[j] = w.hu[i]; hv[j] = w.hv[i];
    live += seq[j] != 0;
  }
  uint32_t total;
  uint32_t o = block_scan_incl(live, w.wsum, tid, &total) - live;
#pragma unroll
  for (int j = 0; j < kWinPer; ++j) if (seq[j] != 0) { win_put(w, o, sal[j], seq[j], e[j], u[j], v[j], hu[j], hv[j]); ++o; }
  if (tid == 0) w.n = total;
  full_barrier();
  return total;
}

__device__ __forceinline__ void win_push_global(const WinState& st, uint32_t e, uint32_t cell) {
  const uint32_t old = atomicExch(&st.whead[cell], e);
  st.er[e].next = old;
  atomicAdd(&st.wcnt[cell], 1u);
}

__device__ __forceinline__ void win_flush(const WinState& st, WinShared& w, int tid) {
  const double smin = st.wrange[0], scale = st.wrange[1];
  if (tid == 0) w.maxcell = 0;
  full_barrier();
  const uint32_t n = w.n < st.wcap ? w.n : st.wcap;
  uint32_t mc = 0;
  for (uint32_t i = tid; i < n; i += kGreedyThreads) {
    if (w.seq[i] == 0) continue;
    const uint32_t c = win_cell(w.sal[i], smin, scale, st.wB);
    win_push_global(st, w.e[i], c);
    mc = mc > c + 1u ? mc : c + 1u;
  }
  if (mc) atomicMax(&w.maxcell, mc);
  full_barrier();
  if (tid == 0) {
    if (w.maxcell && (int)w.maxcell - 1 >= w.cthr) { w.cthr = (int)w.maxcell - 1; w.tsal = __builtin_inf(); w.tseq = ~0ull; }
    w.n = 0;
  }
  full_barrier();
}

__device__ __forceinline__ void win_evict(const WinState& st, WinShared& w, int tid) {
  const double smin = st.wrange[0], scale = st.wrange[1];
// ... 432 lines not shown
```

glia_amd/csrc/hmt_internal.hpp:

```cpp
#pragma once
#include <hip/hip_runtime.h>
#include <stdint.h>
#include <string>
#include <vector>

#include "../../include/glia_hmt.h"

namespace glia {

void set_error(const std::string& msg);
bool option(const char* key, std::string* value = nullptr);
unsigned long long internal_errors();
void count_internal_error();
bool merge_order_is_consistent(const uint32_t* dense_order, int64_t n, uint32_t R, int64_t* first_bad);
int finish_merge_order(int rc, const uint32_t* dense_order, int64_t n, uint32_t R, hipStream_t stream);
#define GLIA_HIP_TRY(expr)                                                                       \
  do {                                                                                           \
    hipError_t _e = (expr);                                                                      \
    if (_e != hipSuccess) {                                                                      \
      ::glia::set_error(std::string(#expr) + ": " + hipGetErrorString(_e));                      \
      return GLIA_HMT_ERR_HIP;                                                                   \
    }                                                                                            \
  } while (0)

constexpr int kTileX = 64;
#ifndef GLIA_ACC_TILEY
#define GLIA_ACC_TILEY 24
#endif
constexpr int kTileY = GLIA_ACC_TILEY;
constexpr int kTZ = 32;

constexpr int R_CNT = 0, R_BORDER = 1, R_LO = 2 , R_HI = 5 , R_SUM = 8 ,
              R_SQ = 10 , R_MIN = 12 , R_MAX = 13 , R_FIRST = 14 , R_HIST = 16;
constexpr int kRegionWords = 32;
constexpr int P_CNT = 0, P_MIN = 1, P_MAX = 2, P_THR = 4 , P_SUM = 8, P_SQ = 10, P_HIST = 12;
constexpr int kPairWords = 32;


struct HistSpec {
  int bins;
  float fb[GLIA_HMT_MAX_BINS];
  float lo_f;
  float hi_f;
};

struct AccParams {
  const uint32_t* lab;
  const uint32_t* lab_c;
  int masked;
  const float* img;
  int64_t nx, ny, nz;
  int64_t gz0, gnz;
  int64_t zb, ze;
  int dim;
  int nbx, nby, nbz;
  int tz;
  HistSpec hist;
  int nthr;
  float thr_f[GLIA_HMT_MAX_THRESH];
  uint32_t* rkeys;
  uint32_t* rrec;
  uint32_t rmask;
  unsigned long long* pkeys;
  uint32_t* prec;
  uint32_t pmask;
  uint32_t* flags;
  uint32_t debug;
};

constexpr int kMaxChannels = 4;
constexpr int kMaxListed = GLIA_HMT_MAX_IMAGES;

struct RagArrays {
  int64_t R = 0, P = 0;
  uint32_t* d_rlabel = nullptr;
  uint32_t* d_rrec = nullptr;
  uint32_t* d_pa = nullptr;
  uint32_t* d_pb = nullptr;
  uint32_t* d_prec = nullptr;
  int K = 1;
  uint32_t* c_rrec[kMaxChannels] = {nullptr, nullptr, nullptr, nullptr};
  uint32_t* c_prec[kMaxChannels] = {nullptr, nullptr, nullptr, nullptr};
  int c_bins[kMaxChannels] = {0, 0, 0, 0};
  unsigned long long* d_pv_off = nullptr;
  float* d_pv = nullptr;
  unsigned long long nV = 0;
};

int launch_accumulate(const AccParams& p, hipStream_t stream);
int launch_synth(int dim, const int64_t dims[3], int S, int G, uint64_t seed, int variant, uint32_t* d_labels,
                 uint32_t* d_truth_tmp, float* d_pb, hipStream_t stream);
constexpr uint32_t kMaskedLabel = 0xFFFFFFFFu;
int launch_mask_fold(const uint32_t* lab, const uint32_t* mask, uint32_t* out, int64_t n, hipStream_t stream);

struct VolumeRef {
  const uint32_t* lab = nullptr;
  const uint32_t* lab_nb = nullptr;
  const float* pb = nullptr;
  int dim = 3;
  long long nx = 1, ny = 1, nz = 1;
  long long zb = 0, ze = -1;
};
struct MedianFeatIn {
  const RagArrays* rag; VolumeRef vol;
  int n_r; const float* r_img[GLIA_HMT_MAX_IMAGES]; int n_b; const float* b_img[GLIA_HMT_MAX_IMAGES];
  const uint32_t* forced; int64_t n_merges;
};
int median_feature_stats(const MedianFeatIn& in, hipStream_t stream, std::vector<double>* reg, std::vector<double>* bnd, std::vector<unsigned long long>* area);
struct TruthCount { uint32_t leaf, truth; unsigned long long count; };
int truth_overlap(const VolumeRef& vol, const uint32_t* d_rlabel, uint32_t R, const uint32_t* d_truth, hipStream_t stream,
                  std::vector<TruthCount>* out, float* ms);
struct NodeTruthStats { std::vector<unsigned long long> n, size, Q; std::vector<long double> E; };
void node_truth_stats(const std::vector<TruthCount>& cnt, uint32_t R, const uint32_t* forced, int64_t M, NodeTruthStats* out, int64_t* moves,
                      int64_t* node_pairs);
int bc_label_rules(const std::vector<NodeTruthStats>& st, uint32_t R, const uint32_t* forced, int64_t M, const glia_hmt_bc_label_opts& o,
                   int32_t* labels);
struct MergeResult {
  std::vector<uint32_t> order;
  std::vector<double> sal, rows;
  int64_t n = 0, n_scored = 0;
  double ms_table = 0.0, ms_init = 0.0, ms_loop = 0.0;
};
struct PbRequest {
  int cond_n = 0;
  long long cond_sizes[2] = {0, 0};
  double cond_rpb = 0.0;
  const VolumeRef* median_of = nullptr;
  bool size_weight = false;
};
int greedy_mean(const RagArrays& rag, hipStream_t stream, const PbRequest& req, MergeResult* out);
struct BcCfg;
struct DeviceClassifier;
struct BcRequest {
  const uint32_t* forced = nullptr;
  int64_t n_forced = 0;
  bool rows = false;
  bool init_only = false;
  bool scores = false;
  int shard = 0, n_shards = 1;
};
#define GLIA_DECLARE_GREEDY_BC(name) \
  int name(const RagArrays& rag, const BcCfg& cfg, const DeviceClassifier& clf, hipStream_t stream, const BcRequest& req, MergeResult* out)
GLIA_DECLARE_GREEDY_BC(greedy_bc_generic);
GLIA_DECLARE_GREEDY_BC(greedy_bc_fma);
GLIA_DECLARE_GREEDY_BC(greedy_bc_sse2);
GLIA_DECLARE_GREEDY_BC(greedy_bc_fma_common);
GLIA_DECLARE_GREEDY_BC(greedy_bc_sse2_common);
GLIA_DECLARE_GREEDY_BC(greedy_bc);
int compact_tables(const AccParams& p, uint32_t rcap, uint32_t pcap, RagArrays* out, hipStream_t stream);
int transform_keys(const uint32_t* order, int64_t n, std::vector<uint32_t>* src, std::vector<uint32_t>* dst);
int transform_image(uint32_t* d_lab, int64_t n, const uint32_t* h_src, const uint32_t* h_dst, int64_t m, const uint32_t* d_mask,
                    int fill_missing, hipStream_t stream, double* ms);
int relabel_image(uint32_t* d_lab, int64_t n, int64_t min_size, uint32_t* n_labels, hipStream_t stream);
int paint_pair_values(const VolumeRef& vol, const uint32_t* d_pa, const uint32_t* d_pb, int64_t P, const float* h_val, float* d_out,
                      hipStream_t stream);
int boundary_confidence_values(int n_trees, const int64_t* n_nodes, const uint32_t* const* node_label, const int32_t* const* parent,
                               const int32_t* const* child0, const double* const* potential, const uint32_t* pa, const uint32_t* pb,
                               int64_t P, std::vector<float>* out);
int watershed_labels(int dim, const int64_t dims[3], const float* d_img, double level, uint32_t* d_out, uint32_t* n_labels, int* sweeps,
                     hipStream_t stream);
int launch_libm_eval(int function, int variant, const double* d_in, double* d_out, int64_t n, hipStream_t stream);
int merge_rag_arrays(const RagArrays* parts, int n_parts, RagArrays* out, hipStream_t stream);
int collect_pair_values(RagArrays* rag, const VolumeRef& vol, hipStream_t stream);
int gather_value_runs(const unsigned long long* src_off, const float* src_vals, const uint32_t* order, uint32_t n, unsigned long long** out_off,
                      float** out_vals, unsigned long long* nV, hipStream_t stream);
int rag_cut_flags(const RagArrays& rag, const uint32_t* d_lab, int64_t nx, int64_t ny, int64_t nzl, int64_t zb, int64_t ze,
                  uint8_t* d_rflag, uint8_t* d_pflag, hipStream_t stream);

__host__ __device__ inline uint32_t float_ord(float f) {
  uint32_t u = __builtin_bit_cast(uint32_t, f);
  return u ^ ((u >> 31) ? 0xFFFFFFFFu : 0x80000000u);
}
__host__ __device__ inline float ord_float(uint32_t o) {
  uint32_t u = o ^ ((o >> 31) ? 0x80000000u : 0xFFFFFFFFu);
  return __builtin_bit_cast(float, u);
}

}
```

glia_amd/hmt.py:

```python
import ctypes as C
import os

import numpy as np

_HERE = os.path.dirname(os.path.abspath(__file__))
_SO = os.environ.get("GLIA_HMT_LIB", os.path.join(_HERE, "libglia_hmt.so"))

MAX_IMAGES, MAX_BINS, MAX_THRESH = 8, 16, 4


class HmtError(RuntimeError):
    def __init__(self, code, msg):
        super().__init__("glia_hmt error %d: %s" % (code, msg))
        self.code = code


class Image(C.Structure):
    _fields_ = [("d_image", C.c_void_p), ("bins", C.c_int), ("lo", C.c_double), ("hi", C.c_double)]


class FeatConfig(C.Structure):
    _fields_ = [
        ("n_region", C.c_int), ("region", Image * MAX_IMAGES),
        ("n_rlabel", C.c_int), ("rlabel", Image * MAX_IMAGES),
# ... 470 lines not shown
        R, P = self.num_regions, self.num_pairs
        rw, pw = C.c_int(), C.c_int()
        _check(lib().glia_hmt_rag_device_arrays(self.h, None, None, None, None, None, C.byref(rw), C.byref(pw)))
        t = dict(rlabel=torch.empty(R, dtype=torch.int32, device=dev), rrec=torch.empty((R, rw.value), dtype=torch.int32, device=dev),
                 pa=torch.empty(P, dtype=torch.int32, device=dev), pb=torch.empty(P, dtype=torch.int32, device=dev),
                 prec=torch.empty((P, pw.value), dtype=torch.int32, device=dev))
        _check(lib().glia_hmt_rag_copy_arrays(self.h, *[C.c_void_p(t[k].data_ptr()) for k in ("rlabel", "rrec", "pa", "pb", "prec")]))
        for k in range(1, lib().glia_hmt_rag_num_channels(self.h)):
            t["rrec%d" % k] = torch.empty((R, rw.value), dtype=torch.int32, device=dev)
            t["prec%d" % k] = torch.empty((P, pw.value), dtype=torch.int32, device=dev)
            _check(lib().glia_hmt_rag_copy_channel(self.h, C.c_int(k), C.c_void_p(t["rrec%d" % k].data_ptr()), C.c_void_p(t["prec%d" % k].data_ptr())))
        return t

    def cut_flags(self, labels_slab, z_begin, z_end):
        import torch
        dev = torch.device("cuda", self.ctx.device)
        _, d = _dims(tuple(labels_slab.shape))
        rcut = torch.zeros(max(self.num_regions, 1), dtype=torch.uint8, device=dev)
        pcut = torch.zeros(max(self.num_pairs, 1), dtype=torch.uint8, device=dev)
        _fence(labels_slab)
        _check(lib().glia_hmt_rag_cut_flags(self.ctx.h, self.h, d, C.c_int64(z_begin), C.c_int64(z_end), C.c_void_p(labels_slab.data_ptr()),
                                            C.c_void_p(rcut.data_ptr()), C.c_void_p(pcut.data_ptr())))
        return rcut[:self.num_regions].bool(), pcut[:self.num_pairs].bool()

    @staticmethod
    def from_tensors(ctx, like, t):
        h = C.c_void_p()
        for k in t:
            assert t[k].is_cuda and t[k].is_contiguous()
        _fence(t["rlabel"])
        _check(lib().glia_hmt_rag_from_arrays(ctx.h, like.h, C.c_int64(t["rlabel"].numel()), C.c_void_p(t["rlabel"].data_ptr()),
                                              C.c_void_p(t["rrec"].data_ptr()), C.c_int64(t["pa"].numel()),
                                              C.c_void_p(t["pa"].data_ptr()), C.c_void_p(t["pb"].data_ptr()),
                                              C.c_void_p(t["prec"].data_ptr()), C.byref(h)))
        k = 1
        while "rrec%d" % k in t:
            _check(lib().glia_hmt_rag_add_channel(ctx.h, h, C.c_void_p(t["rrec%d" % k].data_ptr()), C.c_void_p(t["prec%d" % k].data_ptr())))
            k += 1
        return RegionMap(ctx, None, cfg=like.cfg, _handle=h)

    def last_pass(self):
        ms, by = C.c_double(), C.c_double()
        _check(lib().glia_hmt_rag_last_pass(self.h, C.byref(ms), C.byref(by)))
        return ms.value, by.value

    def regions(self):
        n = self.num_regions
        out = dict(label=np.empty(n, np.uint32), count=np.empty(n, np.int64), border=np.empty(n, np.int64),
                   lo=np.empty((n, 3), np.int64), hi=np.empty((n, 3), np.int64), sum=np.empty(n), sumsq=np.empty(n),
                   min=np.empty(n), max=np.empty(n), hist=np.empty((n, self.bins), np.int64),
                   first=np.empty(n, np.int64))
        _check(lib().glia_hmt_rag_export_regions(self.h, *[_np(out[k]) for k in (
            "label", "count", "border", "lo", "hi", "sum", "sumsq", "min", "max", "hist", "first")]))
        return out

    def pairs(self):
        n = self.num_pairs
        out = dict(a=np.empty(n, np.uint32), b=np.empty(n, np.uint32), count=np.empty(n, np.int64), sum=np.empty(n),
                   sumsq=np.empty(n), min=np.empty(n), max=np.empty(n), hist=np.empty((n, self.bins), np.int64),
                   thr=np.empty((n, max(self.nthr, 1)), np.int64))
        _check(lib().glia_hmt_rag_export_pairs(self.h, *[_np(out[k]) for k in (
            "a", "b", "count", "sum", "sumsq", "min", "max", "hist")], _np(out["thr"]) if self.nthr else None))
        return out

    def merge_order_pb(self, type=1):
        cap = max(self.num_regions, 1)
        order = np.empty((cap, 3), np.uint32)
        sal = np.empty(cap, np.float64)
        n = C.c_int64(0)
        _check(lib().glia_hmt_merge_order_pb(self.ctx.h, self.h, C.c_int(type), _np(order), _np(sal), C.c_int64(cap),
                                             C.byref(n)))
        return order[:n.value].copy(), sal[:n.value].copy()

    def feat_dim(self):
        return lib().glia_hmt_feat_dim(self.h)

    def merge_order_bc(self, classifier, want_feats=False):
        cap = max(self.num_regions, 1)
        order = np.empty((cap, 3), np.uint32)
        sal = np.empty(cap, np.float64)
        d = self.feat_dim()
        feats = np.empty((cap, d), np.float64) if want_feats else None
        n = C.c_int64(0)
        _check(lib().glia_hmt_merge_order_bc(self.ctx.h, self.h, classifier.h, _np(order), _np(sal), _np(feats),
                                             C.c_int64(cap), C.byref(n)))
        if want_feats:
            return order[:n.value].copy(), sal[:n.value].copy(), feats[:n.value].copy()
        return order[:n.value].copy(), sal[:n.value].copy()

    def pre_merge(self, size_thresholds, rpb_threshold):
        cap = max(self.num_regions, 1)
        order = np.empty((cap, 3), np.uint32)
        sal = np.empty(cap, np.float64)
        st = (C.c_int * len(size_thresholds))(*size_thresholds)
        n = C.c_int64(0)
        _check(lib().glia_hmt_pre_merge(self.ctx.h, self.h, st, C.c_int(len(size_thresholds)), C.c_double(rpb_threshold),
                                        _np(order), _np(sal), C.c_int64(cap), C.byref(n)))
        return order[:n.value].copy(), sal[:n.value].copy()

    def bc_feat(self, order, saliencies=None, init_sal=1.0, sal_bias=1.0):
        order = np.ascontiguousarray(order, dtype=np.uint32)
        d = lib().glia_hmt_bc_feat_dim(self.h, C.c_int(1 if saliencies is not None else 0))
        feats = np.empty((len(order), d), np.float64)
        sal = None if saliencies is None else np.ascontiguousarray(saliencies, dtype=np.float64)
        _check(lib().glia_hmt_bc_feat_saliency(self.ctx.h, self.h, _np(order), C.c_int64(len(order)), _np(sal),
                                               C.c_double(init_sal), C.c_double(sal_bias), _np(feats)))
        return feats

    BC_METRICS = {"f1": 0, "ri": 1, "vi": 2}

    def bc_label(self, truths, order, metric="f1", tweak=False, mpd=1.0, opt_split=False, opt=0):
        if not isinstance(truths, (list, tuple)):
            truths = [truths]
        for t in truths:
            assert t.is_cuda and t.is_contiguous() and t.element_size() == 4
            _fence(t)
        order = np.ascontiguousarray(order, dtype=np.uint32).reshape(-1, 3)
        ptrs = (C.c_void_p * max(len(truths), 1))(*[t.data_ptr() for t in truths])
        opts = BcLabelOpts(self.BC_METRICS[metric], int(bool(tweak)), float(mpd), int(bool(opt_split)), int(opt))
        out = np.empty(max(len(order), 1), np.int32)
        _check(lib().glia_hmt_bc_label(self.ctx.h, self.h, ptrs, C.c_int(len(truths)), _np(order), C.c_int64(len(order)),
                                       C.byref(opts), _np(out)))
        return out[:len(order)].copy()

    def last_bc_label_timing(self):
        t = BcLabelTiming()
        _check(lib().glia_hmt_last_bc_label_timing(self.h, C.byref(t)))
        return {k: getattr(t, k) for k, _ in BcLabelTiming._fields_}

    def score_initial_edges(self, classifier):
        n, ms = C.c_int64(0), C.c_double(0)
        _check(lib().glia_hmt_score_initial_edges(self.ctx.h, self.h, classifier.h, C.byref(n), C.byref(ms)))
        return n.value, ms.value

    def score_initial_edges_shard(self, classifier, shard, n_shards):
        cap = max(self.num_pairs, 1)
        out = np.empty(cap, np.float64)
        n = C.c_int64(0)
        _check(lib().glia_hmt_score_initial_edges_shard(self.ctx.h, self.h, classifier.h, C.c_int(shard), C.c_int(n_shards), _np(out),
                                                        C.c_int64(cap), C.byref(n)))
        return out[:n.value].copy()

    def boundary_confidence(self, trees):
        import torch
        nt = len(trees)
        keep = [[np.ascontiguousarray(t[0], np.uint32), np.ascontiguousarray(t[1], np.int32), np.ascontiguousarray(t[2], np.int32),
                 np.ascontiguousarray(t[4], np.float64)] for t in trees]
        nn = (C.c_int64 * nt)(*[len(k[0]) for k in keep])
        arr = lambda j: (C.c_void_p * nt)(*[k[j].ctypes.data for k in keep])
        out = torch.empty(self.shape, dtype=torch.float32, device=torch.device("cuda", self.ctx.device))
        _check(lib().glia_hmt_boundary_confidence(self.ctx.h, self.h, C.c_int(nt), nn, arr(0), arr(1), arr(2), arr(3), C.c_void_p(out.data_ptr())))
        return out

    def last_merge_timing(self):
        a, b, c, n = C.c_double(), C.c_double(), C.c_double(), C.c_int64()
        _check(lib().glia_hmt_last_merge_timing(self.h, C.byref(a), C.byref(b), C.byref(c), C.byref(n)))
        return dict(ms_table=a.value, ms_init=b.value, ms_loop=c.value, n_edges_scored=n.value)
```

include/glia_hmt.h:

```cpp
#ifndef GLIA_HMT_H
#define GLIA_HMT_H

#include <stdint.h>

#ifdef __cplusplus
extern "C" {
#endif

#define GLIA_HMT_OK 0
#define GLIA_HMT_ERR_ARG (-1)
#define GLIA_HMT_ERR_HIP (-2)
#define GLIA_HMT_ERR_UNSUPPORTED (-3)
#define GLIA_HMT_ERR_CAPACITY (-4)
#define GLIA_HMT_ERR_SALIENCY (-5)
#define GLIA_HMT_ERR_IO (-6)
#define GLIA_HMT_ERR_INTERNAL (-7)

#define GLIA_HMT_MAX_IMAGES 8
#define GLIA_HMT_MAX_BINS 16
#define GLIA_HMT_MAX_THRESH 4

typedef struct glia_hmt_ctx glia_hmt_ctx;
typedef struct glia_hmt_rag glia_hmt_rag;
typedef struct glia_hmt_forest glia_hmt_forest;
// ... 25 lines not shown
} glia_hmt_image;

typedef struct {
  int n_region;  glia_hmt_image region[GLIA_HMT_MAX_IMAGES];
  int n_rlabel;  glia_hmt_image rlabel[GLIA_HMT_MAX_IMAGES];
  int n_boundary; glia_hmt_image boundary[GLIA_HMT_MAX_IMAGES];
  const float* d_pb;
  int n_thresholds;
  double thresholds[GLIA_HMT_MAX_THRESH];
  double normalizing_area;
  double normalizing_length;
  int use_log_shape;
  int use_simple_features;
  int use_histogram_features;
  int use_median_features;
} glia_hmt_feat_config;

int glia_hmt_rag_build(glia_hmt_ctx* ctx, int dim, const int64_t dims[3], const uint32_t* d_labels,
                       const uint32_t* d_mask, int only_contour, const float* d_pb,
                       const glia_hmt_feat_config* cfg, glia_hmt_rag** out);
int glia_hmt_rag_build_slab(glia_hmt_ctx* ctx, const int64_t dims_local[3], int64_t z_global_of_plane0,
                            int64_t nz_global, int64_t z_begin, int64_t z_end, const uint32_t* d_labels,
                            int only_contour, const float* d_pb, const glia_hmt_feat_config* cfg, glia_hmt_rag** out);
int glia_hmt_rag_merge(glia_hmt_ctx* ctx, glia_hmt_rag* const* parts, int n_parts, glia_hmt_rag** out);
typedef struct glia_hmt_comm glia_hmt_comm;
int glia_hmt_comm_unique_id(void* id128);
int glia_hmt_comm_create_rccl(glia_hmt_ctx* ctx, int world, int rank, const void* id128, glia_hmt_comm** out);
int glia_hmt_comm_create_local(glia_hmt_ctx* ctx, int world, glia_hmt_comm** out);
void glia_hmt_comm_destroy(glia_hmt_comm* comm);
int glia_hmt_comm_world(const glia_hmt_comm* comm);
int glia_hmt_comm_local_ranks(const glia_hmt_comm* comm, int* ranks, int capacity);
int glia_hmt_slab_range(int64_t nz, int world, int rank, int64_t* first_plane, int64_t* n_planes, int64_t* z_begin, int64_t* z_end);
typedef struct {
  int64_t dims_local[3];
  int64_t z_global_of_plane0;
  int64_t z_begin, z_end;
  const uint32_t* d_labels;
  const float* d_pb;
  const glia_hmt_feat_config* cfg;
} glia_hmt_slab;
typedef struct {
  uint64_t records, cut_records;
  uint64_t bytes_cut_exchange, bytes_to_loop_owner;
} glia_hmt_dist_stats;
int glia_hmt_rag_build_distributed(glia_hmt_ctx* ctx, glia_hmt_comm* comm, const glia_hmt_slab* slabs, int64_t nz_global, int only_contour,
                                   int with_values, int loop_owner, glia_hmt_rag** out, glia_hmt_dist_stats* stats);
int glia_hmt_rag_cut_flags(glia_hmt_ctx* ctx, const glia_hmt_rag* rag, const int64_t dims_local[3], int64_t z_begin, int64_t z_end,
                           const uint32_t* d_labels, uint8_t* d_region_cut, uint8_t* d_pair_cut);
int glia_hmt_rag_device_arrays(const glia_hmt_rag* rag, const uint32_t** d_region_label, const uint32_t** d_region_rec,
                               const uint32_t** d_pair_a, const uint32_t** d_pair_b, const uint32_t** d_pair_rec,
                               int* region_words, int* pair_words);
int glia_hmt_rag_copy_arrays(const glia_hmt_rag* rag, uint32_t* d_region_label, uint32_t* d_region_rec,
                             uint32_t* d_pair_a, uint32_t* d_pair_b, uint32_t* d_pair_rec);
int glia_hmt_rag_from_arrays(glia_hmt_ctx* ctx, const glia_hmt_rag* like, int64_t n_regions,
                             const uint32_t* d_region_label, const uint32_t* d_region_rec, int64_t n_pairs,
                             const uint32_t* d_pair_a, const uint32_t* d_pair_b, const uint32_t* d_pair_rec,
                             glia_hmt_rag** out);
int glia_hmt_rag_num_channels(const glia_hmt_rag* rag);
int glia_hmt_rag_copy_channel(const glia_hmt_rag* rag, int channel, uint32_t* d_region_rec, uint32_t* d_pair_rec);
int glia_hmt_rag_add_channel(glia_hmt_ctx* ctx, glia_hmt_rag* rag, const uint32_t* d_region_rec, const uint32_t* d_pair_rec);
void glia_hmt_rag_free(glia_hmt_rag* rag);
int64_t glia_hmt_rag_num_regions(const glia_hmt_rag* rag);
int64_t glia_hmt_rag_num_pairs(const glia_hmt_rag* rag);
int glia_hmt_rag_export_regions(const glia_hmt_rag* rag, uint32_t* h_label, int64_t* h_count,
                                int64_t* h_border, int64_t* h_bbox_lo , int64_t* h_bbox_hi,
                                double* h_sum, double* h_sumsq, double* h_min, double* h_max,
                                int64_t* h_hist , int64_t* h_first_voxel);
int glia_hmt_rag_export_pairs(const glia_hmt_rag* rag, uint32_t* h_a, uint32_t* h_b, int64_t* h_count,
                              double* h_sum, double* h_sumsq, double* h_min, double* h_max,
                              int64_t* h_hist , int64_t* h_thr );
int glia_hmt_rag_last_pass(const glia_hmt_rag* rag, double* ms, double* algorithmic_bytes);

int glia_hmt_merge_order_pb(glia_hmt_ctx* ctx, glia_hmt_rag* rag, int type, uint32_t* h_order,
                            double* h_saliency, int64_t capacity, int64_t* n_merges);

int glia_hmt_forest_load(glia_hmt_ctx* ctx, int n_models, const char* const* paths, int predict_label,
                         const double* distributor_args , glia_hmt_forest** out);
int glia_hmt_forest_file_parse(const char* path, int predict_label, int* ntree, int* nrnodes, int* nclass,
                               double* h_split, int* h_meta, int64_t capacity_nodes);
int glia_hmt_forest_stub(glia_hmt_ctx* ctx, int feature_index, glia_hmt_forest** out);
void glia_hmt_forest_free(glia_hmt_forest* forest);

int glia_hmt_feat_dim(const glia_hmt_rag* rag);

int glia_hmt_merge_order_bc(glia_hmt_ctx* ctx, glia_hmt_rag* rag, const glia_hmt_forest* forest, uint32_t* h_order,
                            double* h_saliency, double* h_feats, int64_t capacity, int64_t* n_merges);

int glia_hmt_pre_merge(glia_hmt_ctx* ctx, glia_hmt_rag* rag, const int* size_thresholds, int n_thresholds,
                       double rpb_threshold, uint32_t* h_order, double* h_saliency, int64_t capacity, int64_t* n_merges);

int glia_hmt_bc_feat(glia_hmt_ctx* ctx, glia_hmt_rag* rag, const uint32_t* h_order, int64_t n_merges, double* h_feats);
int glia_hmt_bc_feat_saliency(glia_hmt_ctx* ctx, glia_hmt_rag* rag, const uint32_t* h_order, int64_t n_merges,
                              const double* h_saliencies, double init_saliency, double saliency_bias, double* h_feats);
int glia_hmt_bc_feat_dim(const glia_hmt_rag* rag, int with_saliency);

enum { GLIA_HMT_BC_LABEL_F1 = 0, GLIA_HMT_BC_LABEL_RI = 1, GLIA_HMT_BC_LABEL_VI = 2 };
#define GLIA_HMT_BC_MERGE (-1)
#define GLIA_HMT_BC_SPLIT 1
typedef struct {
  int metric;
  int tweak;
  double max_prec_drop;
  int opt_split;
  int global_opt;
} glia_hmt_bc_label_opts;
int glia_hmt_bc_label(glia_hmt_ctx* ctx, glia_hmt_rag* rag, const uint32_t* const* d_truth, int n_truth, const uint32_t* h_order,
                      int64_t n_merges, const glia_hmt_bc_label_opts* opts, int32_t* h_labels);
typedef struct {
  double ms_count;
  double ms_nodes;
  double ms_rules;
  int64_t entries;
  int64_t moves;
  int64_t node_pairs;
} glia_hmt_bc_label_timing;
int glia_hmt_last_bc_label_timing(const glia_hmt_rag* rag, glia_hmt_bc_label_timing* out);

int64_t glia_hmt_tree_potentials(const uint32_t* h_order, int64_t n_merges, const double* h_merge_probs,
                                 const double* h_region_probs, uint32_t* node_label, int32_t* parent, int32_t* child0,
                                 int32_t* child1, double* potential, int64_t capacity);
int64_t glia_hmt_resolve_tree_greedy(const int32_t* parent, const int32_t* child0, const int32_t* child1,
                                     const double* potential, int64_t n_nodes, int32_t* h_picks, int64_t capacity);
int64_t glia_hmt_resolve_trees_greedy(int n_trees, const int64_t* n_nodes, const uint32_t* const* node_label,
                                      const int32_t* const* parent, const int32_t* const* child0, const int32_t* const* child1,
                                      const double* const* potential, int32_t* h_pick_tree, int32_t* h_pick_node, int64_t capacity);
int64_t glia_hmt_label_transform(const uint32_t* node_label, const int32_t* child0, const int32_t* child1, int64_t n_nodes,
                                 const int32_t* h_picks, int64_t n_picks, uint32_t key_to_assign, uint32_t* h_src,
                                 uint32_t* h_dst, int64_t capacity);

int glia_hmt_boundary_confidence(glia_hmt_ctx* ctx, glia_hmt_rag* rag, int n_trees, const int64_t* n_nodes,
                                 const uint32_t* const* node_label, const int32_t* const* parent, const int32_t* const* child0,
                                 const double* const* potential, float* d_out);

int64_t glia_hmt_transform_keys(const uint32_t* h_order, int64_t n_merges, uint32_t* h_src, uint32_t* h_dst, int64_t capacity);

int glia_hmt_transform_image(glia_hmt_ctx* ctx, uint32_t* d_labels, int64_t n_voxels, const uint32_t* h_src,
                             const uint32_t* h_dst, int64_t n_map, const uint32_t* d_mask, int fill_missing);

int glia_hmt_relabel_image(glia_hmt_ctx* ctx, uint32_t* d_labels, int64_t n_voxels, int64_t min_size, uint32_t* n_labels);

double glia_hmt_last_transform_ms(const glia_hmt_ctx* ctx);

int64_t glia_hmt_gen_tree(const uint32_t* h_order, int64_t n_merges, uint32_t* node_label, int32_t* parent,
                          int32_t* child0, int32_t* child1, int64_t capacity);

int glia_hmt_score_initial_edges(glia_hmt_ctx* ctx, glia_hmt_rag* rag, const glia_hmt_forest* forest,
                                 int64_t* n_edges, double* ms);
int glia_hmt_score_initial_edges_shard(glia_hmt_ctx* ctx, glia_hmt_rag* rag, const glia_hmt_forest* forest, int shard,
                                       int n_shards, double* h_scores, int64_t capacity, int64_t* n_records);

int glia_hmt_last_merge_timing(const glia_hmt_rag* rag, double* ms_table, double* ms_init, double* ms_loop,
                               int64_t* n_edges_scored);

int glia_hmt_watershed(glia_hmt_ctx* ctx, int dim, const int64_t dims[3], const float* d_image, double level, uint32_t* d_labels,
                       uint32_t* n_labels, int* sweeps);

int glia_hmt_synth(glia_hmt_ctx* ctx, int dim, const int64_t dims[3], int S, int G, uint64_t seed,
                   int variant, uint32_t* d_labels, float* d_pb);

#ifdef __cplusplus
}
#endif
#endif
```

Baseline: 311,600.

## Split each wave into two half-wave batch members when all candidates are small

The batched greedy merge loop now tracks two candidate keys per wave (one per odd/even lane set), giving 16 candidates instead of 8. When every eligible candidate's adjacency list is small enough, each wave is split into two 32-lane halves, each handling a separate merge with half-size hash tables and bitmap rows. This lets up to 16 merges commit per round instead of 8. It also adds counters for batch statistics exported through a new API. The cost is extra ballots and a larger shared bitmap, plus a more complex selection grid.

```diff
diff --git a/glia_amd/csrc/api.cpp b/glia_amd/csrc/api.cpp
--- a/glia_amd/csrc/api.cpp
+++ b/glia_amd/csrc/api.cpp
@@ -21,7 +21,7 @@
 
 static const char* const kOptionKeys[] = {"GLIA_HMT_PB_WINDOW", "GLIA_HMT_PB_BATCH", "GLIA_HMT_WINCAP", "GLIA_HMT_REBASE", "GLIA_HMT_HORIZON",
                                           "GLIA_HMT_FORCE_TREE", "GLIA_HMT_HELPERS", "GLIA_HMT_TRACE", "GLIA_HMT_LIBM", "GLIA_HMT_BC_NOCOMMON",
-                                          "GLIA_HMT_BC_GENERIC", "GLIA_HMT_DEBUG", "GLIA_HMT_MAXITERS", "GLIA_HMT_MINCAP"};
+                                          "GLIA_HMT_BC_GENERIC", "GLIA_HMT_DEBUG", "GLIA_HMT_MAXITERS", "GLIA_HMT_MINCAP", "GLIA_HMT_BATCH_HALF"};
 static std::mutex g_opt_mu;
 static std::unordered_map<std::string, std::string> g_opt;
 static bool g_opt_init = false;
@@ -755,6 +755,7 @@
   const int rc = greedy_mean(rag->arr, c->stream, req, &res);
   if (rc) return rc;
   rag->ms_table = res.ms_table; rag->ms_loop = res.ms_loop; rag->n_scored = res.n_scored;
+  for (int i = 0; i < 4; ++i) rag->batch_stats[i] = res.batch_stats[i];
   return order_to_keys(rag, res, "merge_order_pb", rag->only_contour, capacity, h_order, h_sal, n_merges);
 }
 
@@ -1269,4 +1270,10 @@
   return GLIA_HMT_OK;
 }
 
-}
+int glia_hmt_last_batch_stats(const glia_hmt_rag* r, int64_t out[4]) {
+  if (!r || !out) return GLIA_HMT_ERR_ARG;
+  for (int i = 0; i < 4; ++i) out[i] = r->batch_stats[i];
+  return GLIA_HMT_OK;
+}
+
+}
diff --git a/glia_amd/csrc/api_types.hpp b/glia_amd/csrc/api_types.hpp
--- a/glia_amd/csrc/api_types.hpp
+++ b/glia_amd/csrc/api_types.hpp
@@ -31,6 +31,7 @@
   double ms_table = 0, ms_init = 0, ms_loop = 0;
   glia_hmt_bc_label_timing bcl;
   int64_t n_scored = 0;
+  int64_t batch_stats[4] = {0, 0, 0, 0};
   glia_hmt_feat_config cfg;
   bool has_cfg = false;
   VolumeRef vol;
diff --git a/glia_amd/csrc/greedy.hip b/glia_amd/csrc/greedy.hip
--- a/glia_amd/csrc/greedy.hip
+++ b/glia_amd/csrc/greedy.hip
@@ -415,6 +415,7 @@
     ws.wcap = kWinCap; ws.wbudget = kWinBudget;
     ws.force_tree = 0;
     if (option("GLIA_HMT_FORCE_TREE", &o_txt)) ws.force_tree = strtoull(o_txt.c_str(), nullptr, 10);
+    ws.batch_half = option("GLIA_HMT_BATCH_HALF", &o_txt) && atoi(o_txt.c_str()) == 0 ? 0u : 1u;
     if (option("GLIA_HMT_WINCAP", &o_txt)) {
       const uint32_t c = (uint32_t)strtoul(o_txt.c_str(), nullptr, 10);
       if (c >= 16 && c <= kWinCap) { ws.wcap = c; ws.wbudget = c / 2; }
@@ -514,6 +515,7 @@
   GLIA_HIP_TRY(hipEventSynchronize(ev.ev[2]));
   out->ms_table = ev.ms(0, 1); out->ms_loop = ev.ms(1, 2);
   out->n_scored = (int64_t)ctrl[CTRL_EDGES];
+  for (int i = 0; i < 4; ++i) out->batch_stats[i] = (int64_t)ctrl[CTRL_BSTAT + i];
   return copy_merges(out, (int64_t)ctrl[CTRL_MERGES], st.order, st.sal_out);
 }
 
diff --git a/glia_amd/csrc/greedy_batch.hpp b/glia_amd/csrc/greedy_batch.hpp
--- a/glia_amd/csrc/greedy_batch.hpp
+++ b/glia_amd/csrc/greedy_batch.hpp
@@ -4,17 +4,20 @@
 namespace glia {
 namespace {
 
-constexpr uint32_t kBatchKill = 32;
+constexpr uint32_t kBatchKill = 64;
 constexpr int kMemP = 3;
 constexpr uint32_t kMemMax = 192;
+constexpr uint32_t kHalfMax = 96;
+constexpr int kNM = 2 * kNW;
+constexpr uint32_t kBmWords = 128;
 struct BatchShared {
-  alignas(16) Key part1[kNW];
-  alignas(16) Key part2[kNW];
+  alignas(16) Key part1[kNM];
+  alignas(16) Key part2[kNM];
   uint32_t nkill, kovf; alignas(16) uint32_t kill[kBatchKill];
-  uint32_t byrank[kNW];
-  uint32_t bitmap[kNW][64];
-  uint32_t m_newcount[kNW], m_total[kNW], m_ok[kNW];
-  double m_maxsal[kNW];
+  uint32_t byrank[kNM];
+  alignas(16) uint32_t bitmap[kNM][kBmWords];
+  uint32_t m_newcount[kNM], m_total[kNM];
+  double m_maxsal[kNM];
   uint32_t bad;
 };
 
@@ -37,6 +40,7 @@
 
 #ifdef GLIA_HMT_PROFILE
 __device__ unsigned long long g_scanprof[8];
+__device__ unsigned long long g_bhist_m[kNM + 1], g_bhist_v[kNM + 1], g_bhist_total[4], g_bkovf;
 __device__ unsigned long long g_scanfill[3][3];
 #define SCAN_T(i) do { if (tid == 0) { const unsigned long long tn_ = __builtin_readcyclecounter(); g_scanprof[i] += tn_ - st_; st_ = tn_; } } while (0)
 #else
@@ -52,7 +56,7 @@
 #ifdef GLIA_HMT_PROFILE
   if (tid == 0) g_scanfill[from][n <= 512u ? 0 : n <= 1024u ? 1 : 2] += 1;
 #endif
-  const uint32_t own = 64u * (uint32_t)(((tid >> 6) + (tid & 63)) & 7) + (uint32_t)(tid & 63);
+  const uint32_t own = 64u * (uint32_t)(((tid >> 6) + ((tid & 63) >> 1)) & 7) + (uint32_t)(tid & 63);
   Key k1, k2;
   k1.sal = -__builtin_inf(); k1.seq = 0; k1.arg = 0; k2 = k1;
   auto pass = [&](auto nb_tag) {
@@ -78,6 +82,9 @@
         for (int j = 0; j < NB; ++j) deadm[j] |= (uint32_t)(kt == e[j]);
       }
       if (kovf) {
+#ifdef GLIA_HMT_PROFILE
+        if (tid == 0) g_bkovf += 1;
+#endif
         full_barrier();
 #pragma unroll
         for (int j = 0; j < NB; ++j) {
@@ -106,42 +113,46 @@
   SCAN_T(1);
   const int lane = tid & 63;
   const unsigned long long o1 = f64_ord(k1.sal), o2 = f64_ord(k2.sal);
-  unsigned long long M1 = o1, M2 = o2;
-  wave_top2_ord(M1, M2);
-  const unsigned long long t1 = __ballot(o1 == M1), t1l = __ballot((o1 == M1) & (k1.seq != 0ull));
-  const int l1 = (int)__builtin_ctzll(t1);
-  const bool win1 = lane == l1;
-  Key kk; kk.sal = win1 ? k2.sal : k1.sal; kk.seq = win1 ? k2.seq : k1.seq; kk.arg = win1 ? k2.arg : k1.arg;
-  const unsigned long long oc = win1 ? o2 : o1;
-  const unsigned long long t2 = __ballot(oc == M2), t2l = __ballot((oc == M2) & (kk.seq != 0ull));
-  Key m1, m2;
-  if (__popcll(t1) == 1 || t1l == 0ull) {
-    m1 = lane_key(k1, l1);
-    int src = (int)__builtin_ctzll(t2);
-    if (__popcll(t2) != 1 && t2l != 0ull) {
-#ifdef GLIA_HMT_PROFILE
-      if (tid == 0) g_scanprof[5] += 1;
-#endif
-      const unsigned long long ms = wave_max_u64(oc == M2 ? kk.seq : 0ull);
-      src = (int)__builtin_ctzll(__ballot((oc == M2) & (kk.seq == ms)));
-    }
-    m2 = lane_key(kk, src);
-    SCAN_T(2);
-  } else {
-#ifdef GLIA_HMT_PROFILE
-    if (tid == 0) g_scanprof[6] += 1;
-#endif
-    unsigned long long S1 = o1 == M1 ? k1.seq : 0ull, S2 = o2 == M1 ? k2.seq : 0ull;
-    wave_top2_ord(S1, S2);
-    const int w1 = (int)__builtin_ctzll(__ballot((o1 == M1) & (k1.seq == S1)));
-    const bool winr = lane == w1;
-    Key kc; kc.sal = winr ? k2.sal : k1.sal; kc.seq = winr ? k2.seq : k1.seq; kc.arg = winr ? k2.arg : k1.arg;
-    const unsigned long long occ = winr ? o2 : o1;
-    m1 = lane_key(k1, w1);
-    m2 = lane_key(kc, (int)__builtin_ctzll(__ballot((occ == M1) & (kc.seq == S2))));
-    SCAN_T(3);
+#pragma nounroll
+  for (int set = 0; set < 2; ++set) {
+    const bool in = (lane & 1) == set;
+    unsigned long long M1 = in ? o1 : 0ull, M2 = in ? o2 : 0ull;
+    wave_top2_ord(M1, M2);
+    const unsigned long long t1 = __ballot(in & (o1 == M1)), t1l = __ballot(in & (o1 == M1) & (k1.seq != 0ull));
+    const int l1 = (int)__builtin_ctzll(t1);
+    const bool win1 = lane == l1;
+    Key kk; kk.sal = win1 ? k2.sal : k1.sal; kk.seq = win1 ? k2.seq : k1.seq; kk.arg = win1 ? k2.arg : k1.arg;
+    const unsigned long long oc = win1 ? o2 : o1;
+    const unsigned long long t2 = __ballot(in & (oc == M2)), t2l = __ballot(in & (oc == M2) & (kk.seq != 0ull));
+    Key m1, m2;
+    if (__popcll(t1) == 1 || t1l == 0ull) {
+      m1 = lane_key(k1, l1);
+      int src = (int)__builtin_ctzll(t2);
+      if (__popcll(t2) != 1 && t2l != 0ull) {
+#ifdef GLIA_HMT_PROFILE
+        if (tid == 0) g_scanprof[5] += 1;
+#endif
+        const unsigned long long ms = wave_max_u64((in & (oc == M2)) ? kk.seq : 0ull);
+        src = (int)__builtin_ctzll(__ballot(in & (oc == M2) & (kk.seq == ms)));
+      }
+      m2 = lane_key(kk, src);
+      SCAN_T(2);
+    } else {
+#ifdef GLIA_HMT_PROFILE
+      if (tid == 0) g_scanprof[6] += 1;
+#endif
+      unsigned long long S1 = (in & (o1 == M1)) ? k1.seq : 0ull, S2 = (in & (o2 == M1)) ? k2.seq : 0ull;
+      wave_top2_ord(S1, S2);
+      const int w1 = (int)__builtin_ctzll(__ballot(in & (o1 == M1) & (k1.seq == S1)));
+      const bool winr = lane == w1;
+      Key kc; kc.sal = winr ? k2.sal : k1.sal; kc.seq = winr ? k2.seq : k1.seq; kc.arg = winr ? k2.arg : k1.arg;
+      const unsigned long long occ = winr ? o2 : o1;
+      m1 = lane_key(k1, w1);
+      m2 = lane_key(kc, (int)__builtin_ctzll(__ballot(in & (occ == M1) & (kc.seq == S2))));
+      SCAN_T(3);
+    }
+    if (lane == 0) { b.part1[2 * (tid >> 6) + set] = m1; b.part2[2 * (tid >> 6) + set] = m2; }
   }
-  if ((tid & 63) == 0) { b.part1[tid >> 6] = m1; b.part2[tid >> 6] = m2; }
   full_barrier();
   SCAN_T(4);
   if (tid == 0) { b.nkill = 0; b.kovf = 0; }
@@ -235,18 +246,20 @@
   uint32_t status = ST_RUN;
   win_enter(st, w, s, tid);
   if (tid == 0) { b.nkill = 0; b.kovf = 0; b.bad = 0; }
-  b.bitmap[wave][lane] = 0;
-  if (tid < kNW) { Key z; z.sal = -__builtin_inf(); z.seq = 0; z.arg = 0; b.part1[tid] = z; b.part2[tid] = z; }
+  for (uint32_t i = tid; i < (uint32_t)kNM * kBmWords; i += kGreedyThreads) b.bitmap[0][i] = 0;
+  if (tid < kNM) b.byrank[tid] = 0;
+  if (tid < kNM) { Key z; z.sal = -__builtin_inf(); z.seq = 0; z.arg = 0; b.part1[tid] = z; b.part2[tid] = z; }
   full_barrier();
   const double smin = st.wrange[0], scale = st.wrange[1];
   uint32_t pend_e = kNone, pend_old = kNone;
   constexpr uint32_t kTab = kMarkSlots / kNW;
-  uint32_t* const tk = &s.mk[wave * kTab]; uint32_t* const t0 = &s.mv0[wave * kTab]; uint32_t* const t1 = &s.mv1[wave * kTab];
+  static_assert(kTab == 256 && kNW == 8, "batch geometry: hash shifts, 16 x 16 selection grid");
   static_assert(sizeof(s.stage) >= (size_t)kNW * kTab * 20, "per-wave staging");
-  uint32_t* const sg_eid = reinterpret_cast<uint32_t*>(&s.stage[0]) + wave * kTab;
-  uint32_t* const sg_n = reinterpret_cast<uint32_t*>(&s.stage[0]) + (kNW + wave) * kTab;
-  uint32_t* const sg_pos = reinterpret_cast<uint32_t*>(&s.stage[0]) + (2 * kNW + wave) * kTab;
-  double* const sg_mean = reinterpret_cast<double*>(reinterpret_cast<uint32_t*>(&s.stage[0]) + 3 * kNW * kTab) + wave * kTab;
+  uint32_t* const sg_eid = reinterpret_cast<uint32_t*>(&s.stage[0]);
+  uint32_t* const sg_n = sg_eid + kNW * kTab;
+  uint32_t* const sg_pos = sg_eid + 2 * kNW * kTab;
+  double* const sg_mean = reinterpret_cast<double*>(sg_eid + 3 * kNW * kTab);
+  uint32_t c_rounds = 0, c_members = 0, c_over8 = 0, c_half = 0;
 #ifdef GLIA_HMT_PROFILE
   unsigned long long bph[8] = {0, 0, 0, 0, 0, 0, 0, 0}, blast = __builtin_readcyclecounter(), brounds = 0, bmembers = 0, bvalid = 0, bwide = 0, bcut_sal = 0, bcut_dep = 0;
   unsigned long long bw_n[4] = {0, 0, 0, 0}, bw_cyc[4] = {0, 0, 0, 0}, bw_ent[4] = {0, 0, 0, 0}, bw_new[4] = {0, 0, 0, 0};
@@ -260,15 +273,24 @@
 
   for (unsigned long long it = 0; it < st.max_iters; ++it) {
     if (ne - st.ne_base > st.rebase_after) { status = ST_REBASE; break; }
-    const int gi = lane >> 3, gj = lane & 7;
-    const Key A = b.part1[gi], B = b.part1[gj], C = b.part2[gi];
-    const unsigned long long beats = __ballot(better(A, B)), under = __ballot(better(C, B));
-    const unsigned long long col = 0x0101010101010101ull << gj;
-    const uint32_t rank = (uint32_t)__popcll(beats & col);
-    const bool cand_ok = B.seq != 0 && (under & col) == 0;
-    if (gi == 0 && cand_ok) b.byrank[rank] = (uint32_t)gj;
-    const unsigned long long okmask = __ballot(gi == 0 && cand_ok);
-    const uint32_t M = (uint32_t)__popcll(okmask);
+    const int gj = lane & 15, gq = lane >> 4;
+    const bool lead = lane < kNM;
+    const Key B = b.part1[gj];
+    uint32_t rank = 0;
+    unsigned long long under = 0;
+    const unsigned long long col = 0x0001000100010001ull << gj;
+#pragma unroll
+    for (int t = 0; t < 4; ++t) {
+      const Key A = b.part1[gq + 4 * t], C = b.part2[gq + 4 * t];
+      rank += (uint32_t)__popcll(__ballot(better(A, B)) & col);
+      under |= __ballot(better(C, B));
+    }
+    const bool cand_ok = lead & (B.seq != 0) & ((under & col) == 0);
+    const uint2 bh0 = w.hu[B.arg], bh1 = w.hv[B.arg];
+    const uint32_t btot = bh0.y + bh1.y;
+    if (cand_ok) b.byrank[rank] = (uint32_t)gj;
+    const uint32_t okmask = (uint32_t)__ballot(cand_ok);
+    const uint32_t M = (uint32_t)__popc(okmask);
     if (M == 0) {
       BPH(5);
       if (pend_e != kNone) { st.er[pend_e].next = pend_old; pend_e = kNone; }
@@ -281,9 +303,15 @@
       batch_scan(st, w, b, tid, kScanOther);
       continue;
     }
-    const unsigned long long minemask = __ballot(gi == 0 && cand_ok && rank == (uint32_t)wave);
+    const bool half = st.batch_half != 0u && (uint32_t)__ballot(cand_ok & (btot > kHalfMax)) == 0u;
+    const uint32_t Mr = half ? M : (M < (uint32_t)kNW ? M : (uint32_t)kNW);
+    const uint32_t hs = half ? (uint32_t)lane >> 5 : 0u, ml = half ? (uint32_t)lane & 31u : (uint32_t)lane, mstride = half ? 32u : 64u;
+    const uint32_t mr = half ? 2u * (uint32_t)wave + hs : (uint32_t)wave;
+    const unsigned long long setmask = half ? 0xFFFFFFFFull << (lane & 32) : ~0ull;
+    const uint32_t mine = (uint32_t)__ballot(cand_ok & (rank == mr - hs)), mine_hi = (uint32_t)__ballot(cand_ok & (rank == mr - hs + 1u));
+    const uint32_t minemask = hs ? mine_hi : mine;
     const bool member = minemask != 0;
-    const int cj = member ? (int)__builtin_ctzll(minemask) : 0;
+    const int cj = member ? (int)__builtin_ctz(minemask) : 0;
     const Key me = b.part1[cj];
     const uint32_t slot = me.arg;
     const uint32_t e = w.e[slot], r0 = w.u[slot], r1 = w.v[slot];
@@ -291,10 +319,9 @@
     const uint32_t off0 = h0r.x, len0 = h0r.y, off1 = h1r.x, len1 = h1r.y;
     const uint32_t total = len0 + len1;
     if (k >= (unsigned long long)st.R0) { status = ST_INTERNAL; break; }
-    const unsigned long long firstmask = __ballot(gi == 0 && cand_ok && rank == 0u);
-    const Key top = b.part1[__builtin_ctzll(firstmask)];
-    const uint2 th0 = w.hu[top.arg], th1 = w.hv[top.arg];
-    const uint32_t top_total = th0.y + th1.y;
+    const int toplane = (int)__builtin_ctz((uint32_t)__ballot(cand_ok & (rank == 0u)));
+    Key top; top.sal = __longlong_as_double((long long)lane_u64((unsigned long long)__double_as_longlong(B.sal), toplane)); top.seq = 0; top.arg = (uint32_t)__builtin_amdgcn_readlane((int)B.arg, toplane);
+    const uint32_t top_total = (uint32_t)__builtin_amdgcn_readlane((int)btot, toplane);
     BPH0(top_total > kMemMax ? 1 : 0);
     if (top_total > kMemMax) {
       if (ne + top_total > st.Ecap) { status = ST_NEED_EDGES; break; }
@@ -315,14 +342,17 @@
       BPH(4);
       continue;
     }
-    const bool narrow = member && total <= kMemMax;
-    b.bitmap[wave][lane] = 0;
+    const bool narrow = member & (total <= (half ? kHalfMax : kMemMax));
+    const uint32_t brow = 2u * (uint32_t)wave + hs;
+    *reinterpret_cast<uint4*>(&b.bitmap[2 * wave + (lane >> 5)][4 * (lane & 31)]) = make_uint4(0u, 0u, 0u, 0u);
+    const uint32_t tb = (uint32_t)wave * kTab + hs * (kTab / 2u), tmask = half ? kTab / 2u - 1u : kTab - 1u, tshift = half ? 25u : 24u;
+    uint32_t* const tk = &s.mk[tb]; uint32_t* const t0 = &s.mv0[tb]; uint32_t* const t1 = &s.mv1[tb];
     FatEntry fe[kMemP];
     bool act[kMemP], side1[kMemP];
     uint32_t h[kMemP];
 #pragma unroll
     for (int p = 0; p < kMemP; ++p) {
-      const uint32_t i = (uint32_t)lane + 64u * (uint32_t)p;
+      const uint32_t i = ml + mstride * (uint32_t)p;
       const bool inlist = narrow && i < total;
       side1[p] = i >= len0;
       fe[p].eid = kNone; fe[p].rs = 0; fe[p].n = 0; fe[p].pos = 0; fe[p].off = 0; fe[p].len = 0; fe[p].mean = 0.0;
@@ -333,21 +363,21 @@
 #pragma unroll
     for (int p = 0; p < kMemP; ++p) {
       act[p] = act[p] && fe[p].eid != e && fe[p].eid != kNone;
-      h[p] = (fe[p].rs * 2654435761u) >> 24;
+      h[p] = (fe[p].rs * 2654435761u) >> tshift;
       if (act[p]) {
         while (true) {
           const uint32_t old = atomicCAS(&tk[h[p]], 0u, fe[p].rs + 1u);
           if (old == 0u || old == fe[p].rs + 1u) break;
-          h[p] = (h[p] + 1u) & (kTab - 1u);
+          h[p] = (h[p] + 1u) & tmask;
         }
         if (side1[p]) {
           t1[h[p]] = 1u;
-          sg_eid[h[p]] = fe[p].eid; sg_n[h[p]] = fe[p].n; sg_pos[h[p]] = fe[p].pos; sg_mean[h[p]] = fe[p].mean;
+          sg_eid[tb + h[p]] = fe[p].eid; sg_n[tb + h[p]] = fe[p].n; sg_pos[tb + h[p]] = fe[p].pos; sg_mean[tb + h[p]] = fe[p].mean;
         } else t0[h[p]] = 1u;
-        atomicOr(&b.bitmap[wave][(fe[p].rs >> 5) & 63u], 1u << (fe[p].rs & 31u));
-      }
-    }
-    if (narrow && lane == 0) { atomicOr(&b.bitmap[wave][(r0 >> 5) & 63u], 1u << (r0 & 31u)); atomicOr(&b.bitmap[wave][(r1 >> 5) & 63u], 1u << (r1 & 31u)); }
+        atomicOr(&b.bitmap[brow][(fe[p].rs >> 5) & (kBmWords - 1u)], 1u << (fe[p].rs & 31u));
+      }
+    }
+    if (narrow && ml == 0u) { atomicOr(&b.bitmap[brow][(r0 >> 5) & (kBmWords - 1u)], 1u << (r0 & 31u)); atomicOr(&b.bitmap[brow][(r1 >> 5) & (kBmWords - 1u)], 1u << (r1 & 31u)); }
     asm volatile("s_waitcnt lgkmcnt(0)" ::: "memory");
     bool owner[kMemP], both[kMemP];
     uint32_t p_eid[kMemP], p_n[kMemP], p_pos[kMemP];
@@ -357,7 +387,7 @@
       const uint32_t m0 = act[p] ? t0[h[p]] : 0u, m1 = act[p] ? t1[h[p]] : 0u;
       owner[p] = act[p] && (!side1[p] || m0 == 0u);
       both[p] = owner[p] && !side1[p] && m1 != 0u;
-      p_eid[p] = sg_eid[h[p]]; p_n[p] = sg_n[h[p]]; p_pos[p] = sg_pos[h[p]]; p_mean[p] = sg_mean[h[p]];
+      p_eid[p] = sg_eid[tb + h[p]]; p_n[p] = sg_n[tb + h[p]]; p_pos[p] = sg_pos[tb + h[p]]; p_mean[p] = sg_mean[tb + h[p]];
     }
 #pragma unroll
     for (int p = 0; p < kMemP; ++p) if (act[p]) { tk[h[p]] = 0u; t0[h[p]] = 0u; t1[h[p]] = 0u; }
@@ -370,14 +400,14 @@
       const bool h0 = owner[p] && !side1[p], h1 = owner[p] && (side1[p] || both[p]);
       bad = mean_link(h0, fe[p].mean, (int)fe[p].n, h1, both[p] ? p_mean[p] : fe[p].mean, both[p] ? (int)p_n[p] : (int)fe[p].n, &first[p], &second[p]) || bad;
       const double f = first[p];
-      const unsigned long long ownmask = __ballot(owner[p]);
+      const unsigned long long ownmask = __ballot(owner[p]) & setmask;
       idx[p] = newcount + (uint32_t)__popcll(ownmask & ((1ull << lane) - 1ull));
       newcount += (uint32_t)__popcll(ownmask);
       mx = (owner[p] && -f > mx) ? -f : mx;
     }
 #pragma unroll
-    for (int d = 32; d >= 1; d >>= 1) { const double o = __shfl_xor(mx, d); mx = o > mx ? o : mx; }
-    if (lane == 0) { b.m_newcount[wave] = narrow ? newcount : 0u; b.m_total[wave] = narrow ? total : 0xFFFFFFFFu; b.m_maxsal[wave] = mx; }
+    for (int d = 32; d >= 1; d >>= 1) { const double o = __shfl_xor(mx, d); mx = ((o > mx) & ((uint32_t)d < mstride)) ? o : mx; }
+    if (ml == 0u) { b.m_newcount[mr] = narrow ? newcount : 0u; b.m_total[mr] = narrow ? total : 0xFFFFFFFFu; b.m_maxsal[mr] = mx; }
     if (bad) b.bad = 1;
     const uint32_t wn_round = w.n;
     lds_barrier();
@@ -385,26 +415,32 @@
     if (b.bad) { status = ST_BAD_SALIENCY; break; }
     uint32_t V, ne_off, pool_off, my_ne, my_pool;
     {
-      const uint32_t j = (uint32_t)lane & 7u;
-      const Key kj = b.part1[b.byrank[j]];
+      const uint32_t j = (uint32_t)lane & 15u, q = (uint32_t)lane >> 4;
+      const Key kj = b.part1[b.byrank[j] & 15u];
       const uint32_t u = w.u[kj.arg], v = w.v[kj.arg];
       const uint32_t tj = b.m_total[j], nj = b.m_newcount[j];
       double pm = -__builtin_inf();
       uint32_t hit = 0, pre_n = 0, pre_t = 0;
 #pragma unroll
-      for (uint32_t i = 0; i < (uint32_t)kNW; ++i) {
+      for (uint32_t t = 0; t < 4u; ++t) {
+        const uint32_t i = 4u * q + t, row = half ? i : (2u * i) & 15u;
         const double ms = b.m_maxsal[i];
-        const uint32_t bu = b.bitmap[i][(u >> 5) & 63u], bv = b.bitmap[i][(v >> 5) & 63u];
+        const uint32_t bu = b.bitmap[row][(u >> 5) & (kBmWords - 1u)], bv = b.bitmap[row][(v >> 5) & (kBmWords - 1u)];
         const uint32_t ti = b.m_total[i], ni = b.m_newcount[i];
-        if (i < j) { pm = ms > pm ? ms : pm; hit |= ((bu >> (u & 31u)) | (bv >> (v & 31u))) & 1u; pre_n += ni; pre_t += ti; }
-      }
-      const bool okj = j < M && tj != 0xFFFFFFFFu && (j == 0u || (kj.sal > pm && hit == 0u));
-      const uint32_t okbits = (uint32_t)(__ballot(lane < kNW && okj) & 0xFFull);
+        const bool before = i < j;
+        pm = (before & (ms > pm)) ? ms : pm; hit |= before ? ((bu >> (u & 31u)) | (bv >> (v & 31u))) & 1u : 0u; pre_n += before ? ni : 0u; pre_t += before ? ti : 0u;
+      }
+      const unsigned long long fine = __ballot((kj.sal > pm) & (hit == 0u));
+      const uint32_t fine4 = (uint32_t)(fine & (fine >> 16) & (fine >> 32) & (fine >> 48)) & 0xFFFFu;
+      const bool okj = (j < Mr) & (tj != 0xFFFFFFFFu) & ((j == 0u) | (((fine4 >> j) & 1u) != 0u));
+      const uint32_t okbits = (uint32_t)__ballot(lead & okj);
       V = (uint32_t)__builtin_ctz(~okbits);
 #ifdef GLIA_HMT_PROFILE
-      if (V < M) { const uint32_t cutsal = (uint32_t)(__ballot(lane < kNW && j == V && !(kj.sal > pm)) & 0xFFull); if (cutsal) bcut_sal += 1; else bcut_dep += 1; }
-#endif
-      my_ne = (uint32_t)__builtin_amdgcn_readlane((int)pre_n, wave); my_pool = (uint32_t)__builtin_amdgcn_readlane((int)pre_t, wave);
+      if (V < Mr) { if (__ballot((j == V) & !(kj.sal > pm))) bcut_sal += 1; else bcut_dep += 1; }
+#endif
+      pre_n += (uint32_t)__shfl_xor((int)pre_n, 16); pre_n += (uint32_t)__shfl_xor((int)pre_n, 32);
+      pre_t += (uint32_t)__shfl_xor((int)pre_t, 16); pre_t += (uint32_t)__shfl_xor((int)pre_t, 32);
+      my_ne = (uint32_t)__shfl((int)pre_n, (int)mr); my_pool = (uint32_t)__shfl((int)pre_t, (int)mr);
       const uint32_t last = V - 1u;
       ne_off = (uint32_t)__shfl((int)(pre_n + nj), (int)last); pool_off = (uint32_t)__shfl((int)(pre_t + tj), (int)last);
     }
@@ -413,24 +449,27 @@
     if (pool_used + sum_tot > st.pool_cap) { status = ST_NEED_POOL; break; }
     bool popped = false;
     if (wn_round + ne_off > st.wcap && wn_round > st.wcap / 2u) {
-      if ((uint32_t)wave < V && lane == 0) w.seq[slot] = 0;
+      if ((mr < V) & (ml == 0u)) w.seq[slot] = 0;
       popped = true;
       lds_barrier();
       win_compact(w, tid, st.wcap);
     }
     const WinTau tau = {w.cthr, w.tsal, w.tseq, smin, scale};
     BPH(2);
-    if ((uint32_t)wave < V) {
-      const unsigned long long kk = k + (unsigned long long)wave;
+    if (mr < V) {
+      const unsigned long long kk = k + (unsigned long long)mr;
       const uint32_t r2 = st.R0 + (uint32_t)kk;
       const uint32_t r2off = (uint32_t)pool_used + my_pool;
-      if (lane == 0) {
+      if (ml == 0u) {
         if (!popped) w.seq[slot] = 0;
         st.order[3 * kk + 0] = r0; st.order[3 * kk + 1] = r1; st.order[3 * kk + 2] = r2;
         st.sal_out[kk] = me.sal;
         st.er[e].seq = 0;
         st.rdead[r0] = 1; st.rdead[r1] = 1;
         st.adj_off[r2] = r2off; st.adj_len[r2] = newcount;
+#ifdef GLIA_HMT_PROFILE
+        atomicAdd(&g_bhist_total[total <= 32u ? 0 : total <= 64u ? 1 : total <= 96u ? 2 : 3], 1ull);
+#endif
       }
 #pragma unroll
       for (int p = 0; p < kMemP; ++p) {
@@ -452,7 +491,9 @@
     BPH(3);
 #ifdef GLIA_HMT_PROFILE
     brounds += 1; bmembers += M; bvalid += V;
-#endif
+    if (tid == 0) { g_bhist_m[M] += 1; g_bhist_v[V] += 1; }
+#endif
+    c_rounds += 1u; c_members += V; c_over8 += V > 8u ? 1u : 0u; c_half += half ? 1u : 0u;
     k += V; ne += ne_off; pool_used += pool_off;
     batch_scan(st, w, b, tid, kScanNarrow);
     if (w.spill_ord) { if (pend_e != kNone) { st.er[pend_e].next = pend_old; pend_e = kNone; } win_evict(st, w, tid); batch_scan(st, w, b, tid, kScanOther); }
@@ -465,6 +506,14 @@
                        g_scanprof[0], g_scanprof[1], g_scanprof[2], g_scanprof[3], g_scanprof[4], g_scanprof[7], g_scanprof[5], g_scanprof[6]);
   if (tid == 0) printf("[batch profile] scan fill (cumulative; n <= 512, <= 1024, more): after reload/evict %llu %llu %llu  after narrow round %llu %llu %llu  after wide %llu %llu %llu\n",
                        g_scanfill[0][0], g_scanfill[0][1], g_scanfill[0][2], g_scanfill[1][0], g_scanfill[1][1], g_scanfill[1][2], g_scanfill[2][0], g_scanfill[2][1], g_scanfill[2][2]);
+  if (tid == 0) {
+    printf("[batch profile] narrow rounds by candidates M = 1..16 (cumulative):");
+    for (int i = 1; i <= kNM; ++i) printf(" %llu", g_bhist_m[i]);
+    printf("\n[batch profile] narrow rounds by committed members V = 1..16 (cumulative):");
+    for (int i = 1; i <= kNM; ++i) printf(" %llu", g_bhist_v[i]);
+    printf("\n[batch profile] committed members by list entries (<=32, <=64, <=96, <=192; cumulative): %llu %llu %llu %llu  scans on the kovf path %llu  this launch: half-mode rounds %u of %u, rounds that committed more than 8: %u\n",
+           g_bhist_total[0], g_bhist_total[1], g_bhist_total[2], g_bhist_total[3], g_bkovf, c_half, c_rounds, c_over8);
+  }
   if (tid == 0) printf("[batch profile] loop top (this launch): narrow rounds %llu cycles %llu  wide pops %llu cycles %llu\n", bsel_n[0], bsel[0], bsel_n[1], bsel[1]);
   if (tid == 0) printf("[batch profile] wide phases (cumulative cycles): entry-barrier %llu  lists+table %llu  compact %llu  main loop (wave 0) %llu  loop barrier %llu  tail %llu\n",
                        g_wideprof[0], g_wideprof[1], g_wideprof[2], g_wideprof[3], g_wideprof[4], g_wideprof[5]);
@@ -474,7 +523,8 @@
   if (pend_e != kNone) st.er[pend_e].next = pend_old;
   full_barrier();
   win_leave(st, w, tid, k, ne, pool_used, status);
-}
-
-}
-}
+  if (tid == 0) { st.ctrl[CTRL_BSTAT + 0] += c_rounds; st.ctrl[CTRL_BSTAT + 1] += c_members; st.ctrl[CTRL_BSTAT + 2] += c_over8; st.ctrl[CTRL_BSTAT + 3] += c_half; }
+}
+
+}
+}
diff --git a/glia_amd/csrc/greedy_tree.hpp b/glia_amd/csrc/greedy_tree.hpp
--- a/glia_amd/csrc/greedy_tree.hpp
+++ b/glia_amd/csrc/greedy_tree.hpp
@@ -31,7 +31,9 @@
 enum { CTRL_MERGES = 0, CTRL_EDGES = 1, CTRL_ENTRIES = 2,
        CTRL_STATUS = 3, CTRL_VALUES = 4,
        CTRL_CTHR = 5, CTRL_TSAL = 6, CTRL_TSEQ = 7, CTRL_IPTR = 8,
-       CTRL_WERR = 9, CTRL_WFILL = 10, CTRL_WORDS = 11 };
+       CTRL_WERR = 9, CTRL_WFILL = 10,
+       CTRL_BSTAT = 11,
+       CTRL_WORDS = 15 };
 
 namespace {
 
diff --git a/glia_amd/csrc/greedy_window.hpp b/glia_amd/csrc/greedy_window.hpp
--- a/glia_amd/csrc/greedy_window.hpp
+++ b/glia_amd/csrc/greedy_window.hpp
@@ -40,6 +40,7 @@
   uint32_t wch;
   uint8_t* rdead;
   unsigned long long force_tree;
+  uint32_t batch_half;
 };
 constexpr uint32_t kWinCap = 1536;
 constexpr uint32_t kWinBudget = 768;
diff --git a/glia_amd/csrc/hmt_internal.hpp b/glia_amd/csrc/hmt_internal.hpp
--- a/glia_amd/csrc/hmt_internal.hpp
+++ b/glia_amd/csrc/hmt_internal.hpp
@@ -119,6 +119,7 @@
   std::vector<uint32_t> order;
   std::vector<double> sal, rows;
   int64_t n = 0, n_scored = 0;
+  int64_t batch_stats[4] = {0, 0, 0, 0};
   double ms_table = 0.0, ms_init = 0.0, ms_loop = 0.0;
 };
 struct PbRequest {
diff --git a/glia_amd/hmt.py b/glia_amd/hmt.py
--- a/glia_amd/hmt.py
+++ b/glia_amd/hmt.py
@@ -646,6 +646,11 @@
         _check(lib().glia_hmt_boundary_confidence(self.ctx.h, self.h, C.c_int(nt), nn, arr(0), arr(1), arr(2), arr(3), C.c_void_p(out.data_ptr())))
         return out
 
+    def last_batch_stats(self):
+        out = (C.c_int64 * 4)()
+        _check(lib().glia_hmt_last_batch_stats(self.h, out))
+        return dict(rounds=out[0], members=out[1], rounds_over8=out[2], rounds_half=out[3])
+
     def last_merge_timing(self):
         a, b, c, n = C.c_double(), C.c_double(), C.c_double(), C.c_int64()
         _check(lib().glia_hmt_last_merge_timing(self.h, C.byref(a), C.byref(b), C.byref(c), C.byref(n)))
diff --git a/include/glia_hmt.h b/include/glia_hmt.h
--- a/include/glia_hmt.h
+++ b/include/glia_hmt.h
@@ -201,6 +201,8 @@
 int glia_hmt_last_merge_timing(const glia_hmt_rag* rag, double* ms_table, double* ms_init, double* ms_loop,
                                int64_t* n_edges_scored);
 
+int glia_hmt_last_batch_stats(const glia_hmt_rag* rag, int64_t out[4]);
+
 int glia_hmt_watershed(glia_hmt_ctx* ctx, int dim, const int64_t dims[3], const float* d_image, double level, uint32_t* d_labels,
                        uint32_t* n_labels, int* sweeps);
 
```

Result: slower. 297,700 (-4.5%).
